# danihae/bio-image-unet

Measured on AMD Instinct MI355X. Metric: voxels/sec fwd+bwd, higher is better.
Workload: dtype bf16; 1 GPU; cfg4: UNet3D(in_channels=1, out_channels=1, n_filter=32) input (4, 1, 128, 128, 128) per GPU, train step = forward + reference loss + backward + Adam; parallelism=dp1

## Files before the change

bio_image_unet_amd/_lib.py:

```python
from __future__ import annotations

import ctypes as C
import os

import torch

_HERE = os.path.dirname(os.path.abspath(__file__))
LIB_PATH = os.environ.get("BIU_LIB_PATH") or os.path.join(_HERE, "libbiu_hip.so")

BIU_F32, BIU_BF16 = 0, 1
BN_MAX_PARTIALS = 1024


class BiuError(RuntimeError):
    pass


class biu_act(C.Structure):
    _fields_ = [("p", C.c_void_p), ("n", C.c_int32), ("d", C.c_int32), ("h", C.c_int32), ("w", C.c_int32),
                ("c", C.c_int32), ("pitch", C.c_int32)]


class biu_pack_job(C.Structure):
    _fields_ = [("w", C.c_void_p), ("packed", C.c_void_p), ("transposed", C.c_int32), ("kind", C.c_int32), ("cin", C.c_int32),
                ("cout", C.c_int32), ("kd", C.c_int32), ("kh", C.c_int32), ("kw", C.c_int32), ("reserved", C.c_int32)]


class biu_xform(C.Structure):
    _fields_ = [("scale", C.c_void_p), ("shift", C.c_void_p), ("slope", C.c_void_p)]


class biu_mo2d_term(C.Structure):
    _fields_ = [("kind", C.c_int32), ("nb", C.c_int32), ("partial_off", C.c_longlong), ("numel", C.c_longlong), ("pixels", C.c_longlong),
                ("p0", C.c_float), ("p1", C.c_float), ("p2", C.c_float), ("weight", C.c_float)]


class biu_aug_params(C.Structure):
    _fields_ = [("flags", C.c_uint32), ("rot_k", C.c_uint32), ("blur_k", C.c_uint32), ("index", C.c_uint32), ("m", C.c_double * 6),
                ("alpha", C.c_float), ("beta", C.c_float), ("noise_a", C.c_float), ("noise_b", C.c_float),
                ("angle", C.c_float), ("scale", C.c_float), ("dx", C.c_float), ("dy", C.c_float)]


class biu_augf_params(C.Structure):
    _fields_ = [("flags", C.c_uint32), ("rot_k", C.c_uint32), ("blur_k", C.c_uint32), ("index", C.c_uint32), ("m", C.c_double * 6),
                ("cos_t", C.c_float), ("sin_t", C.c_float), ("alpha", C.c_float), ("beta", C.c_float), ("shot_s", C.c_float),
                ("gauss_sigma", C.c_float), ("angle", C.c_float), ("scale", C.c_float), ("dx", C.c_float), ("dy", C.c_float)]


_P = C.c_void_p
_A = C.POINTER(biu_act)
_X = C.POINTER(biu_xform)
_I = C.c_int
_F = C.c_float
_D = C.c_double
_Z = C.c_size_t

SIGNATURES = {
    "biu_last_error": (C.c_char_p, []),
    "biu_version": (_I, []),
    "biu_set_fp32_products": (_I, [_I]),
    "biu_set_fp32_products_3d": (_I, [_I]),
    "biu_conv_packed_bytes": (_Z, [_I, _I, _I, _I, _I, _I, _I, _I]),
    "biu_conv_pack": (_I, [_I, _P, _I, _I, _I, _I, _I, _I, _P, _P]),
    "biu_pack_batch": (_I, [_P, _I, _I, _P]),
    "biu_conv_split_workspace": (_Z, [_I, _A, _A, _I, _I, _I, _I, _I]),
    "biu_conv_fwd": (_I, [_A, _X, _P, _P, _P, _I, _I, _I, _I, _A, _P, _Z, _I, _P]),
    "biu_conv_fwd_stats_floats": (_Z, [_A, _I]),
    "biu_conv_fwd_stats": (_I, [_A, _X, _P, _P, _P, _I, _I, _I, _I, _A, _P, _Z, C.POINTER(C.c_int), _P, _Z, _I, _P]),
    "biu_conv_bwd_data": (_I, [_A, _P, _P, _I, _I, _I, _I, _A, _I, _P, _Z, _I, _P]),
    "biu_bwd_data_bnred_floats": (_Z, [_A, _I, _I]),
    "biu_conv_bwd_data_bnred": (_I, [_A, _P, _P, _I, _I, _I, _I, _A, _A, _P, _P, _P, _P, _P, _P, _Z, C.POINTER(C.c_int), _P, _Z, _I, _P]),
    "biu_convt_bwd_data_bnred": (_I, [_A, _P, _P, _I, _A, _A, _P, _P, _P, _P, _P, _P, _Z, C.POINTER(C.c_int), _I, _P]),
    "biu_conv_bwd_weight_workspace": (_Z, [_I, _I, _I, _I, _I, _I]),
    "biu_conv_bwd_weight": (_I, [_A, _X, _A, _I, _I, _I, _I, _P, _P, _P, _Z, _I, _P]),
    "biu_conv_bwd_weight_bn": (_I, [_A, _X, _A, _A, _P, _P, _P, _P, _P, _P, _I, _I, _I, _I, _P, _P, _Z, _I, _P]),
    "biu_bn_stats": (_I, [_A, _P, C.POINTER(C.c_int), _I, _P]),
    "biu_bn_finalize": (_I, [_P, _I, _I, _D, _P, _P, _P, _P, _F, _F, _P, _P, _P, _P, _P]),
    "biu_bn_eval_affine": (_I, [_I, _P, _P, _P, _P, _F, _P, _P, _P]),
    "biu_xform_apply": (_I, [_A, _X, _A, _I, _P]),
    "biu_bn_bwd_reduce": (_I, [_A, _A, _P, _P, _P, _P, _P, _P, C.POINTER(C.c_int), _I, _P]),
    "biu_bn_bwd_finalize": (_I, [_P, _I, _I, _D, _P, _P, _P, _P, _P, _P, _P, _P, _P]),
    "biu_bn_bwd_finalize_eval": (_I, [_P, _I, _I, _P, _P, _P, _P, _P, _P, _P, _P]),
    "biu_bn_bwd_apply": (_I, [_A, _A, _P, _P, _P, _P, _P, _P, _A, _I, _P]),
    "biu_maxpool_fwd": (_I, [_A, _X, _A, _I, _P]),
    "biu_maxpool_bwd": (_I, [_A, _X, _A, _A, _I, _I, _P]),
    "biu_maxpool_bwd_bnred": (_I, [_A, _X, _A, _A, _I, _P, _P, _P, _Z, C.POINTER(C.c_int), _I, _P]),
    "biu_nearest_down_fwd": (_I, [_A, _X, _A, _I, _P]),
    "biu_nearest_down_bwd": (_I, [_A, _A, _I, _I, _P]),
    "biu_nearest_up_fwd": (_I, [_A, _X, _A, _I, _P]),
    "biu_upconv_ok": (_I, [_A, _A, _I]),
    "biu_upconv_packed_bytes": (_Z, [_I, _I, _I, _I]),
    "biu_upconv_pack": (_I, [_I, _P, _I, _I, _I, _P, _P]),
    "biu_upconv_bwd_data": (_I, [_A, _P, _A, _I, _I, _P]),
    "biu_upconv_bwd_weight_workspace": (_Z, [_I, _I, _I]),
    "biu_upconv_bwd_weight_bn": (_I, [_A, _X, _A, _A, _P, _P, _P, _P, _P, _P, _P, _P, _Z, _I, _P]),
    "biu_upconv_fwd_stats_floats": (_Z, [_A, _A]),
    "biu_upconv_fwd": (_I, [_A, _X, _P, _P, _A, _P, _Z, C.POINTER(C.c_int), _I, _P]),
    "biu_nearest_up_bwd": (_I, [_A, _A, _I, _I, _P]),
    "biu_bce_dice_blocks": (_I, [C.c_longlong]),
    "biu_bce_dice_fwd": (_I, [_P, _P, _I, C.c_longlong, _P, _P]),
    "biu_bce_dice_bwd": (_I, [_P, _P, _I, C.c_longlong, _P, _P, _I, _P]),
    "biu_pair_smooth_l1_blocks": (_I, [C.c_longlong]),
    "biu_pair_smooth_l1_fwd": (_I, [_P, _I, C.c_longlong, _P, _P]),
    "biu_pair_smooth_l1_bwd": (_I, [_P, _I, C.c_longlong, _P, _P, _I, _P]),
    "biu_seg_loss_finish": (_I, [_P, _I, _I, C.c_longlong, _P, _I, _F, _F, _F, _I, _F, _F, _F, _I, _F, _P, _P]),
    "biu_seg_loss_coef": (_I, [_P, _P, _I, C.c_longlong, _F, _F, _F, _I, _F, _F, _F, _I, _F, _P, _P, _P]),
    "biu_head_dlogits": (_I, [_P, _P, _P, _I, _I, _I, C.c_longlong, _P, _I, _I, _P]),
    "biu_mo2d_loss_blocks": (_I, [C.c_longlong]),
    "biu_mo2d_loss_fwd": (_I, [_I, _F, _F, _P, _I, _P, _I, _I, _I, _I, _P, _P]),
    "biu_mo2d_loss_finish": (_I, [_P, _I, _P, _P, _P]),
    "biu_mo2d_loss_coef": (_I, [_P, _I, _P, _P, _P, _P]),
    "biu_mo2d_loss_bwd": (_I, [_I, _F, _F, _P, _I, _P, _I, _I, _I, _I, _P, _P, _P]),
    "biu_trilinear_up_fwd": (_I, [_A, _X, _A, _I, _P]),
    "biu_trilinear_up_bwd": (_I, [_A, _A, _I, _I, _P]),
    "biu_bilinear_up_fwd": (_I, [_A, _X, _A, _I, _P]),
    "biu_bilinear_up_bwd": (_I, [_A, _A, _I, _I, _P]),
    "biu_xcorr_fwd": (_I, [_A, _X, _A, _X, _A, _I, _P]),
    "biu_xcorr_bwd": (_I, [_A, _X, _A, _X, _A, _A, _A, _I, _I, _P]),
    "biu_conv_cat_ok": (_I, [_A, _A, _A, _I, _I, _I, _I, _I]),
    "biu_conv_fwd_cat": (_I, [_A, _X, _A, _X, _P, _P, _P, _I, _I, _I, _I, _A, _P, _Z, C.POINTER(C.c_int), _P, _Z, _I, _P]),
    "biu_conv_bwd_data_cat": (_I, [_A, _P, _P, _I, _I, _I, _I, _A, _I, _A, _I, _P, _Z, _I, _P]),
    "biu_conv_bwd_weight_cat": (_I, [_A, _X, _A, _X, _A, _A, _P, _P, _P, _P, _P, _P, _I, _I, _I, _I, _P, _P, _Z, _I, _P]),
    "biu_convt_packed_bytes": (_Z, [_I, _I, _I, _I, _I]),
    "biu_convt_pack": (_I, [_I, _P, _I, _I, _I, _I, _P, _P]),
    "biu_foldt_ok": (_I, [_A, _A, _A, _I]),
    "biu_foldt_packed_bytes": (_Z, [_I, _I, _I, _I]),
    "biu_foldt_pack": (_I, [_P, _P, _P, _P, _I, _I, _I, _I, _I, _P, _P]),
    "biu_foldt_fwd_stats_floats": (_Z, [_A, _A]),
# ... 94 lines not shown
```

bio_image_unet_amd/csrc/biu_api.hip:

```cpp
#include "biu_common.h"
#include "biu_internal.h"

#include <stdlib.h>
#include <string.h>

static const char* const kOffTokens[] = {
    "conv_fwd", "conv_dgrad", "conv_wgrad", "convt_fwd", "convt_dgrad", "convt_wgrad", "convt_all", "c1", "c1_mfma", "cat",
    "fused_stats", "wgrad_bn", "dgrad_bnred", "pool_pair", "pool_pipe", "pool_bnred", "head_bnred", "ksplit", "m16", "m16x2", "rr16",
    "wroll", "wroll16", "wroll2d", "upconv", "foldt", "foldall", "foldck8", "foldgemm", "croll", "froll", "prepack", "wsplitbn",
    "capturefork", "sidechain",
};
constexpr int kNumOffTokens = sizeof(kOffTokens) / sizeof(kOffTokens[0]);
static_assert(kNumOffTokens <= 64, "BiuEnv::off holds one bit per token");

static int off_index(const char* tok, size_t n) {
    for (int i = 0; i < kNumOffTokens; ++i)
        if (strlen(kOffTokens[i]) == n && strncmp(kOffTokens[i], tok, n) == 0) return i;
    return -1;
}
static void env_unknown(const char* var, const char* val, int n) {
    fprintf(stderr, "[biu] %s: unknown %s '%.*s' ignored\n", var, strcmp(var, "BIU_DISABLE") == 0 ? "token" : "value", n, val);
}
static bool parse_int(const char* s, int* v) {
    char* end = nullptr;
    const long r = strtol(s, &end, 10);
    if (end == s || *end) return false;
    *v = (int)r;
    return true;
}

const BiuEnv& biu_env() {
    static const BiuEnv env = [] {
        BiuEnv v{0, false, false, 0, 2, 0, 128};
        if (const char* p = getenv("BIU_DISABLE")) {
            while (true) {
                const size_t n = strcspn(p, ",");
                const int i = off_index(p, n);
                if (i >= 0) v.off |= 1ull << i;
                else if (n > 0) env_unknown("BIU_DISABLE", p, (int)n);
                if (!p[n]) break;
                p += n + 1;
            }
        }
        if (const char* e = getenv("BIU_ROLL"); e && *e) {
            if (strcmp(e, "always") == 0) v.roll_always = true;
            else env_unknown("BIU_ROLL", e, (int)strlen(e));
        }
        if (const char* e = getenv("BIU_FOLDT"); e && *e) {
            int n = 0;
            if (strcmp(e, "always") == 0) v.foldt_always = true;
            else if (strncmp(e, "cmax:", 5) == 0 && parse_int(e + 5, &n) && n > 0) v.foldt_cmax = n;
            else if (strcmp(e, "size") != 0) env_unknown("BIU_FOLDT", e, (int)strlen(e));
        }
        if (const char* e = getenv("BIU_FP32_PRODUCTS"); e && *e) {
            if (strcmp(e, "exact") == 0) v.fp32_products = 0;
            else if (strcmp(e, "bf16x3") == 0) v.fp32_products = 1;
            else if (strcmp(e, "bf16x6") != 0) env_unknown("BIU_FP32_PRODUCTS", e, (int)strlen(e));
        }
        if (const char* e = getenv("BIU_FP32_PRODUCTS_3D"); e && *e) {
            if (strcmp(e, "bf16x3") == 0) v.fp32_products_3d = 1;
            else if (strcmp(e, "bf16x6") == 0) v.fp32_products_3d = 2;
            else if (strcmp(e, "exact") != 0) env_unknown("BIU_FP32_PRODUCTS_3D", e, (int)strlen(e));
        }
// ... 192 lines not shown
        return a > b ? a : b;
    }
    return biu_mfma_wgrad_workspace(cin, cout, kd, kh, kw, dtype);
}

extern "C" int biu_conv_bwd_weight(const biu_act* x, const biu_xform* xf, const biu_act* dy, int kd, int kh, int kw,
                                   int dilation, float* dw, float* dbias, void* ws, size_t ws_bytes, int dtype,
                                   biu_stream stream) {
    BIU_REQUIRE(conv_args_ok(x, dy, kd, kh, kw, dilation), BIU_ERR_SHAPE, "conv_bwd_weight: x/dy extents differ");
    BIU_REQUIRE(dw, BIU_ERR_SHAPE, "conv_bwd_weight: null dw");
    if (!biu_off("c1") && biu_c1m_ok(x, dy, kd, kh, kw, dilation, dtype) && ws && ws_bytes >= biu_c1m_wgrad_workspace(dy->c, kd)) {
        int rc = biu_c1m_wgrad(x, xf, dy, nullptr, kd, dw, ws, ws_bytes, (hipStream_t)stream);
        if (rc == BIU_OK && dbias) rc = biu_chan_sum(dy, dbias, dtype, (hipStream_t)stream);
        return rc;
    }
    if (!biu_off("c1") && biu_c1_conv_ok(x, dy, kd, kh, kw, dilation, dtype) && ws && ws_bytes >= biu_c1_wgrad_workspace(dy->c, kd)) {
        int rc = biu_c1_conv_wgrad(x, xf, dy, kd, dw, ws, ws_bytes, dtype, (hipStream_t)stream);
        if (rc == BIU_OK && dbias) rc = biu_chan_sum(dy, dbias, dtype, (hipStream_t)stream);
        return rc;
    }
    if (!biu_off("conv_wgrad") && biu_mfma_wgrad_ok(x, dy, kd, kh, kw, dilation, dtype)) {
        BIU_REQUIRE(ws && ws_bytes >= biu_mfma_wgrad_workspace(x->c, dy->c, kd, kh, kw, dtype), BIU_ERR_WORKSPACE,
                    "conv_bwd_weight: workspace too small");
        return biu_mfma_wgrad(x, xf, dy, kd, kh, kw, dw, dbias, ws, ws_bytes, dtype, (hipStream_t)stream);
    }
    warn_slow_path("conv_bwd_weight", x, dy, kd * kh * kw);
    return biu_conv_bwd_weight_direct(x, xf, dy, kd, kh, kw, dilation, dw, dbias, dtype, (hipStream_t)stream);
}

extern "C" int biu_conv_bwd_weight_bn(const biu_act* x, const biu_xform* xf, const biu_act* da, const biu_act* y,
                                      const float* scale, const float* shift, const float* slope, const float* coefA,
                                      const float* coefB, const float* coefC, int kd, int kh, int kw, int dilation,
                                      float* dw, void* ws, size_t ws_bytes, int dtype, biu_stream stream) {
    BIU_REQUIRE(conv_args_ok(x, da, kd, kh, kw, dilation) && valid_act(y) && same_space(y, da) && y->c == da->c, BIU_ERR_SHAPE,
                "conv_bwd_weight_bn: extents differ");
    BIU_REQUIRE(dw && scale && shift && coefA && coefB && coefC, BIU_ERR_SHAPE, "conv_bwd_weight_bn: null pointer");
    const size_t es = dsize(dtype);
    const bool yok = ((uintptr_t)y->p % 16) == 0 && ((size_t)y->pitch * es) % 16 == 0 &&
                     (i64)y->d * y->h * y->w * y->pitch * (i64)es < (1LL << 32) - 65536;
    if (!biu_off("c1") && !biu_off("wgrad_bn") && yok && biu_c1m_ok(x, da, kd, kh, kw, dilation, dtype) && ws &&
        ws_bytes >= biu_c1m_wgrad_workspace(da->c, kd)) {
        BnBwdFuse bn{y, scale, shift, slope, coefA, coefB, coefC};
        return biu_c1m_wgrad(x, xf, da, &bn, kd, dw, ws, ws_bytes, (hipStream_t)stream);
    }
    if (!biu_off("conv_wgrad") && !biu_off("wgrad_bn") && yok && biu_mfma_wgrad_ok(x, da, kd, kh, kw, dilation, dtype)) {
        BIU_REQUIRE(ws && ws_bytes >= biu_mfma_wgrad_workspace(x->c, da->c, kd, kh, kw, dtype), BIU_ERR_WORKSPACE,
                    "conv_bwd_weight_bn: workspace too small");
        BnBwdFuse bn{y, scale, shift, slope, coefA, coefB, coefC};
        return biu_mfma_wgrad(x, xf, da, kd, kh, kw, dw, nullptr, ws, ws_bytes, dtype, (hipStream_t)stream, &bn);
    }
    int rc = biu_bn_bwd_apply(da, y, scale, shift, slope, coefA, coefB, coefC, da, dtype, stream);
    if (rc != BIU_OK) return rc;
    return biu_conv_bwd_weight(x, xf, da, kd, kh, kw, dilation, dw, nullptr, ws, ws_bytes, dtype, stream);
}

extern "C" int biu_conv_cat_ok(const biu_act* x0, const biu_act* x1, const biu_act* y, int kd, int kh, int kw, int dilation, int dtype) {
    if (!x0 || !x1 || !y || !valid_act(x0) || !valid_act(x1) || !valid_act(y) || !same_space(x0, y) || !same_space(x1, y)) return 0;
    if (biu_off("conv_fwd") || biu_off("conv_dgrad") || biu_off("conv_wgrad") || biu_off("cat")) return 0;
    return biu_mfma_conv_cat_ok(x0, x1, y, kd, kh, kw, dilation, dtype) ? 1 : 0;
}
extern "C" int biu_conv_fwd_cat(const biu_act* x0, const biu_xform* xf0, const biu_act* x1, const biu_xform* xf1, const float* w,
                                const void* packed, const float* bias, int kd, int kh, int kw, int dilation, const biu_act* y,
                                float* bn_partial, size_t bn_partial_floats, int* bn_nblk, void* ws, size_t ws_bytes, int dtype,
                                biu_stream stream) {
    BIU_REQUIRE(biu_conv_cat_ok(x0, x1, y, kd, kh, kw, dilation, dtype) && w && packed, BIU_ERR_UNSUPPORTED,
                "conv_fwd_cat: shapes not served by the two-source kernels (ask biu_conv_cat_ok)");
    ConvCat cat{x1, xf1, nullptr, 0};
    if (bn_partial && will_split(x0->c + x1->c, y, nullptr, kd, dtype, ws, ws_bytes)) {
        BIU_REQUIRE(bn_nblk, BIU_ERR_SHAPE, "conv_fwd_cat: null bn_nblk");
        int rc = biu_mfma_conv(x0, xf0, packed, bias, kd, kh, kw, y, 0, nullptr, dtype, (hipStream_t)stream, nullptr, &cat, ws, ws_bytes);
        if (rc != BIU_OK) return rc;
        BIU_REQUIRE(bn_partial_floats >= (size_t)BIU_BN_MAX_PARTIALS * y->c * 2, BIU_ERR_WORKSPACE, "conv_fwd_cat: partial buffer too small");
        return biu_bn_stats(y, bn_partial, bn_nblk, dtype, stream);
    }
    if (bn_partial) {
        BIU_REQUIRE(bn_nblk, BIU_ERR_SHAPE, "conv_fwd_cat: null bn_nblk");
        const int nb = dtype == BIU_F32 ? biu_mfma_conv_stat_rows(y, kd, x0, dtype, false, x0->c + x1->c) : biu_mfma_conv_stat_rows(y, kd);
        BIU_REQUIRE((size_t)nb * y->c * 2 <= bn_partial_floats, BIU_ERR_WORKSPACE, "conv_fwd_cat: partial buffer too small");
        int rc = biu_mfma_conv(x0, xf0, packed, bias, kd, kh, kw, y, 0, bn_partial, dtype, (hipStream_t)stream, nullptr, &cat);
        if (rc == BIU_OK) *bn_nblk = nb;
        return rc;
    }
    return biu_mfma_conv(x0, xf0, packed, bias, kd, kh, kw, y, 0, nullptr, dtype, (hipStream_t)stream, nullptr, &cat, ws, ws_bytes);
}
extern "C" int biu_conv_bwd_data_cat(const biu_act* dy, const float* w, const void* packed, int kd, int kh, int kw, int dilation,
                                     const biu_act* dx0, int accumulate0, const biu_act* dx1, int accumulate1, void* ws, size_t ws_bytes,
                                     int dtype, biu_stream stream) {
    BIU_REQUIRE(biu_conv_cat_ok(dx0, dx1, dy, kd, kh, kw, dilation, dtype) && w && packed, BIU_ERR_UNSUPPORTED,
                "conv_bwd_data_cat: shapes not served by the two-source kernels (ask biu_conv_cat_ok)");
    ConvCat cat{nullptr, nullptr, dx1, accumulate1};
    return biu_mfma_conv(dy, nullptr, packed, nullptr, kd, kh, kw, dx0, accumulate0, nullptr, dtype, (hipStream_t)stream, nullptr, &cat, ws, ws_bytes);
}
extern "C" int biu_conv_bwd_weight_cat(const biu_act* x0, const biu_xform* xf0, const biu_act* x1, const biu_xform* xf1,
                                       const biu_act* da, const biu_act* y, const float* scale, const float* shift,
                                       const float* slope, const float* coefA, const float* coefB, const float* coefC, int kd,
                                       int kh, int kw, int dilation, float* dw, void* ws, size_t ws_bytes, int dtype,
                                       biu_stream stream) {
    BIU_REQUIRE(biu_conv_cat_ok(x0, x1, da, kd, kh, kw, dilation, dtype) && dw, BIU_ERR_UNSUPPORTED,
                "conv_bwd_weight_cat: shapes not served by the two-source kernels (ask biu_conv_cat_ok)");
    BIU_REQUIRE(ws && ws_bytes >= biu_mfma_wgrad_workspace(x0->c + x1->c, da->c, kd, kh, kw, dtype), BIU_ERR_WORKSPACE,
                "conv_bwd_weight_cat: workspace too small");
    if (y) {
        const size_t es = dsize(dtype);
        BIU_REQUIRE(valid_act(y) && same_space(y, da) && y->c == da->c && scale && shift && coefA && coefB && coefC, BIU_ERR_SHAPE,
                    "conv_bwd_weight_cat: BatchNorm operands missing");
        BIU_REQUIRE(((uintptr_t)y->p % 16) == 0 && ((size_t)y->pitch * es) % 16 == 0 && (i64)y->d * y->h * y->w * y->pitch * (i64)es < (1LL << 32) - 65536,
// ... 198 lines not shown
```

bio_image_unet_amd/csrc/biu_conv_mfma.hip:

```cpp
#include "biu_internal.h"
#include <type_traits>
#include <cstring>
#include <mutex>
#include <cstdlib>

typedef float floatx16 __attribute__((ext_vector_type(16)));
typedef float floatx4 __attribute__((ext_vector_type(4)));
typedef __bf16 bf16x8 __attribute__((ext_vector_type(8)));

template <typename T> struct Frag;
template <> struct Frag<bf16_t> {
    static constexpr int PE = 8;
    __device__ static __forceinline__ void mma(const uint4& a, const uint4& b, floatx16& c) {
        c = __builtin_amdgcn_mfma_f32_32x32x16_bf16(__builtin_bit_cast(bf16x8, a), __builtin_bit_cast(bf16x8, b), c, 0, 0, 0);
    }
    __device__ static __forceinline__ void unpack(const uint4& v, float* f) {
        const unsigned u[4] = {v.x, v.y, v.z, v.w};
#pragma unroll
        for (int i = 0; i < 4; ++i) {
            f[2 * i] = __uint_as_float(u[i] << 16);
            f[2 * i + 1] = __uint_as_float(u[i] & 0xffff0000u);
        }
    }
    __device__ static __forceinline__ uint4 pack(const float* f) {
// ... 2262 lines not shown
    if (rc == BIU_OK) rc = mfma_pack_strided(1, w_conv + (size_t)cup * 27, ccat, cskip, cout, 3, 3, 3, dtype, base + b.sdg, st);
    return rc;
}
static bool foldt_roll_ok(const biu_act* x_low, const biu_act* skip, const biu_act* y, int dtype) {
    return !biu_off("froll") && skip && biu_fold_roll_ok(x_low, y, dtype) && biu_conv_roll_ok(skip, y, dtype, false, 1, false);
}
int biu_mfma_foldt_form(const biu_act* x_low, const biu_act* skip, const biu_act* y, int dtype) { return foldt_roll_ok(x_low, skip, y, dtype) ? 1 : 0; }
int biu_mfma_foldt_stat_rows(const biu_act* x_low, const biu_act* y, const biu_act* skip, int dtype) {
    if (skip && foldt_roll_ok(x_low, skip, y, dtype)) return biu_conv_roll_rows(skip, y, dtype);
    return biu_mfma_upconv_stat_rows(x_low, y);
}
int biu_mfma_foldt_fwd(const biu_act* x_low, const biu_xform* xf_low, const biu_act* skip, const biu_xform* xf_skip, const void* packed, const biu_act* y,
                       float* bn_partial, int dtype, hipStream_t st) {
    const FoldtBlob b = foldt_blob(x_low->c, skip->c, y->c, dtype);
    const char* base = (const char*)packed;
    if (foldt_roll_ok(x_low, skip, y, dtype)) {
        int rc = biu_fold_roll(x_low, xf_low, base + b.fwd, (const float*)(base + b.bias), (const float*)(base + b.fix), y, st);
        if (rc != BIU_OK) return rc;
        return biu_mfma_conv(skip, xf_skip, base + b.sfwd, nullptr, 3, 3, 3, y, 1, bn_partial, dtype, st, nullptr, nullptr, nullptr, 0);
    }
    int rc = biu_mfma_conv(skip, xf_skip, base + b.sfwd, (const float*)(base + b.bias), 3, 3, 3, y, 0, nullptr, dtype, st, nullptr, nullptr, nullptr, 0);
    if (rc != BIU_OK) return rc;
    const ShellDims sh = shell_dims(y->n, y->d, y->h, y->w);
    BIU_DISPATCH_DTYPE(dtype, hipLaunchKernelGGL(k_foldt_border_fix<T>, dim3(2048), dim3(256), 0, st, (char*)y->p,
                                                 sh, y->c, y->pitch, (const float*)(base + b.fix)));
    BIU_CHECK_LAUNCH("foldt_border_fix");
    return biu_mfma_upconv_fwd(x_low, xf_low, base + b.fwd, nullptr, y, bn_partial, dtype, st, 1);
}

typedef __bf16 bf16x4 __attribute__((ext_vector_type(4)));

struct WgradArgs {
    const char* pa;
    const char* pb;
    float* ws;
    const float* as_; const float* ab_; const float* al_;
    const float* bs_; const float* bb_; const float* bl_;
    int apitch, bpitch;
    int N, CA, CB;
    int GD, GH, GW;
    int BD, BH, BW;
    int nbd, nbh, nbw, nbricks;
    int njt;
    int jt_begin, jt_count;
    int write_back;
    unsigned long long* diag;
    const char* pb1; int bpitch1; int bsplit;
    const float* bs1_; const float* bb1_; const float* bl1_;
    int bricks_per_block;
    const char* py;
    int ypitch;
    const float* bn_scale; const float* bn_shift; const float* bn_slope;
    const float* bn_cA; const float* bn_cB; const float* bn_cC;
    float* dbias_out;
    int fold_par;
    size_t fold_slice_f;
};

template <typename T, int PE>
__device__ __forceinline__ uint4 apply_xf16(uint4 v, const float* sc, const float* sh, const float* sl) {
    using F = Frag<T>;
    float f[PE];
    F::unpack(v, f);
    lrelu_affine<PE>(f, sc, sh, sl);
    return F::pack(f);
}


constexpr bool wgrad_tab_in_lds(size_t tile_bytes, int pieces) { return tile_bytes + (size_t)pieces * 512 * 4 <= 150 * 1024; }

template <typename T, int KD, int KHW, int S, int TD, int TH, int TW, int KSPLIT, int NI, bool RR16 = false, bool FALL = false>
__global__ __launch_bounds__(512, 2) void k_wgrad_pipe(WgradArgs a) {
    using F = Frag<T>;
    constexpr int NTHR = 512, NWAVE = 8;
    constexpr int PE = F::PE;
    constexpr int CT = 32;
    constexpr int PPV = CT / PE;
    constexpr int XP = SplitOf<T>::parts;
    constexpr bool X3 = XP > 0;
    constexpr bool BFM = sizeof(T) == 2 || X3;
    constexpr int LES = BFM ? 2 : 4;
    constexpr int NPL = X3 ? XP : 1;
    constexpr int CTA = CT * NI, PPVA = CTA / PE, RSA = CTA * LES;
    constexpr int PD = (KD == 3) ? 1 : 0;
    constexpr int PHW = (KHW == 3) ? 1 : 0;
    constexpr bool FOLD = (KD == 2 && KHW == 2 && S == 1);
    constexpr int SD = (KD == 1) ? 1 : S;
    static_assert(!FALL || (FOLD && KSPLIT == 8 && NI == 1 && sizeof(T) == 2), "the all-parity form: bf16 fold, one wave per parity class");
    constexpr int HD = (TD - 1) * SD + (FALL ? 3 : KD), HH = (TH - 1) * S + (FALL ? 3 : KHW), HW = (TW - 1) * S + (FALL ? 3 : KHW);
    constexpr int HV = HD * HH * HW;
    constexpr int BVR = TD * TH * TW;
    constexpr int BV = FALL ? 8 * BVR : BVR;
    constexpr int TAPS = KD * KHW * KHW;
    constexpr int WPQ = NWAVE / KSPLIT;
    constexpr int IPW = (TAPS + WPQ - 1) / WPQ;
    static_assert(NWAVE % KSPLIT == 0, "K split must divide the wave count");
    constexpr int RS = CT * LES;
    constexpr int NA = (BV * PPVA + NTHR - 1) / NTHR;
    constexpr int NB = (HV * PPV + NTHR - 1) / NTHR;
    constexpr int KUNIT = BFM ? 16 : 2;
    constexpr int NKG = BV / KUNIT;
    static_assert(TW % 16 == 0 && NKG % KSPLIT == 0, "brick / split mismatch");

    extern __shared__ __attribute__((aligned(16))) uint4 lds[];
    char* at = (char*)lds;
    char* bt = at + NPL * BV * RSA;
// ... 591 lines not shown
    float* wsp = a.ws + (FALL ? (size_t)wave * a.fold_slice_f : (size_t)0);
    if (jj < a.CB) {
#pragma unroll
        for (int t2 = 0; t2 < IPW; ++t2) {
            const int tap = tapid[t2];
            if (tap < TAPS) {
#pragma unroll
                for (int ni = 0; ni < NI; ++ni)
#pragma unroll
                    for (int e = 0; e < 16; ++e) {
                        const int ii = it * CTA + ni * CT + (e & 3) + 8 * (e >> 2) + 4 * hf;
                        if (ii < a.CA) atomicAdd(wsp + ((size_t)tap * a.CA + ii) * a.CB + jj, acc[t2][ni][e]);
                    }
            }
        }
    }
}

typedef unsigned v4u_t __attribute__((ext_vector_type(4)));
__device__ __forceinline__ void bload_lds16(unsigned voff, v4u_t rsrc, unsigned lds_base_uniform) {
    unsigned keep;
    asm volatile("s_mov_b32 %0, m0\n\ts_mov_b32 m0, %3\n\ts_nop 0\n\tbuffer_load_dwordx4 %1, %2, 0 offen lds\n\ts_mov_b32 m0, %0"
                 : "=&s"(keep)
                 : "v"(voff), "s"(rsrc), "s"(lds_base_uniform)
                 : "memory");
}
__device__ __forceinline__ v4u_t raw_rsrc(const void* base, unsigned bytes) {
    const unsigned long long pa = (unsigned long long)base;
    v4u_t r;
    r[0] = __builtin_amdgcn_readfirstlane((unsigned)pa);
    r[1] = __builtin_amdgcn_readfirstlane((unsigned)(pa >> 32) & 0xffffu);
    r[2] = __builtin_amdgcn_readfirstlane(bytes);
    r[3] = 0x00020000u;
    return r;
}

#ifndef BIU_WROLL_ABL
#define BIU_WROLL_ABL 0
#endif
#ifndef BIU_DIAG_WAVE
#define BIU_DIAG_WAVE 0
#endif
constexpr int WR_TD = 2, WR_TH = 8, WR_TW = 16;
constexpr int WR_HH = WR_TH + 2, WR_HW = WR_TW + 2, WR_PL = WR_HH * WR_HW;
constexpr int WR_RS = 64;
constexpr int WR_PLB = WR_PL * WR_RS;
constexpr int WR_NBI = 24;
constexpr int WR_PAIRB = WR_NBI * 1024;
constexpr int WR_NPAIR = 4;
constexpr int WR_BV = WR_TD * WR_TH * WR_TW;
constexpr int WR_AB = WR_BV * WR_RS;
constexpr int WR_NAI = WR_AB / 1024;
constexpr int WR_NABUF = 3;
constexpr size_t WR_LDS = (size_t)WR_NPAIR * WR_PAIRB + WR_NABUF * WR_AB + 9 * 32 * sizeof(float);

__device__ __forceinline__ unsigned opaque_s(unsigned x) { asm volatile("" : "+s"(x)); return x; }
template <int N> __device__ __forceinline__ void wait_vmcnt() { asm volatile("s_waitcnt vmcnt(%0)" ::"n"(N) : "memory"); }

template <bool BNF, bool K2D, bool A16 = false>
__global__ __launch_bounds__(512, 2) void k_wgrad_roll(WgradArgs a) {
    static_assert(!(K2D && A16), "the 16-channel plain operand form exists for volumes only");
    using T = bf16_t;
    using F = Frag<T>;
    constexpr int TD = WR_TD, TH = WR_TH, TW = WR_TW, HW = WR_HW, PL = WR_PL, RS = WR_RS, PLB = WR_PLB, PAIRB = WR_PAIRB;
    constexpr int CT = 32, PE = 8, TAPS = K2D ? 9 : 27, IPW = K2D ? 3 : 4, NROW = TD * TH;
    constexpr int NBK = WR_NBI / 8, NAK = A16 ? 1 : WR_NAI / 8;
    constexpr int NACC = A16 ? 6 : IPW;

    extern __shared__ __attribute__((aligned(16))) uint4 lds[];
    char* bring = (char*)lds;
    char* abuf = bring + WR_NPAIR * PAIRB;
    float* lxf = (float*)(abuf + WR_NABUF * WR_AB);
    constexpr int LB = 0, LBN = 3 * CT;

    const int tid = threadIdx.x, lane = tid & 63;
    const int wave = __builtin_amdgcn_readfirstlane(tid >> 6);
    const int it = blockIdx.y / a.jt_count, jt = a.jt_begin + blockIdx.y % a.jt_count;
    const int piece = lane & 3;
    const int apc = A16 ? (piece & 1) : piece;
    const int ac0 = it * CT + apc * PE, bc0 = jt * CT + piece * PE;
    const bool apiece_ok = ac0 < a.CA, bpiece_ok = bc0 < a.CB;
    const bool b_src1 = a.pb1 && jt * CT >= a.bsplit;
    const char* pb_ = b_src1 ? a.pb1 : a.pb;
    const int bpitch_ = b_src1 ? a.bpitch1 : a.bpitch;
    const int bc_local = bc0 - (b_src1 ? a.bsplit : 0);
    const float* bs_ = b_src1 ? a.bs1_ : a.bs_;
    const float* bb_ = b_src1 ? a.bb1_ : a.bb_;
    const float* bl_ = b_src1 ? a.bl1_ : a.bl_;
    const bool b_xf = bs_ != nullptr;
    constexpr bool bn_fused = BNF;
    const bool wb = bn_fused && a.write_back;
    if (tid < CT && bn_fused) {
        const int ca = it * CT + tid;
        const bool ok = ca < a.CA;
        lxf[LBN + 0 * CT + tid] = ok ? a.bn_scale[ca] : 1.f;
        lxf[LBN + 1 * CT + tid] = ok ? a.bn_shift[ca] : 0.f;
        lxf[LBN + 2 * CT + tid] = (ok && a.bn_slope) ? a.bn_slope[ca] : 1.f;
        lxf[LBN + 3 * CT + tid] = ok ? a.bn_cA[ca] : 0.f;
        lxf[LBN + 4 * CT + tid] = ok ? a.bn_cB[ca] : 0.f;
        lxf[LBN + 5 * CT + tid] = ok ? a.bn_cC[ca] : 0.f;
    }
    if (tid < CT) {
        const int cb = jt * CT + tid;
        const int cbl = cb - (b_src1 ? a.bsplit : 0);
        lxf[LB + 0 * CT + tid] = (b_xf && cb < a.CB) ? bs_[cbl] : 1.f;
        lxf[LB + 1 * CT + tid] = (b_xf && cb < a.CB) ? bb_[cbl] : 0.f;
        lxf[LB + 2 * CT + tid] = (b_xf && cb < a.CB) ? bl_[cbl] : 1.f;
    }

    floatx16 acc[NACC];
#pragma unroll
    for (int t = 0; t < NACC; ++t)
#pragma unroll
        for (int e = 0; e < 16; ++e) acc[t][e] = 0.f;
    const int wkd = wave / 3, wkw = wave % 3;
    const bool has_x = A16 ? (wave < 4) : (!K2D && wave < 3);
    int tapid[IPW];
#pragma unroll
    for (int t = 0; t < IPW; ++t) {
        if constexpr (K2D) tapid[t] = (wave < 6) ? t * 3 + wkw : TAPS;
        else tapid[t] = (t < 3) ? (wkd * 3 + t) * 3 + wkw : (has_x ? (2 * 3 + wave) * 3 + 2 : TAPS);
    }
    int ab_lane;
    {
        const int g = lane >> 4, li = lane & 15, qrow = li >> 2, p = li & 3, cg = g & 1, h = g >> 1;
        ab_lane = (8 * h + qrow) * RS + (16 * cg + 4 * p) * 2;
    }

    unsigned bco[NBK], aco[NAK];
#pragma unroll
    for (int k = 0; k < NBK; ++k) {
        const int v = ((wave + 8 * k) * 64 + lane) >> 2;
        const int pl = v / PL, r = v % PL;
        bco[k] = (v < 2 * PL && bpiece_ok) ? (unsigned)(pl | ((r / HW) << 10) | ((r % HW) << 20)) : 0xffffffffu;
    }
#pragma unroll
    for (int k = 0; k < NAK; ++k) {
        const int v = ((wave + 8 * k) * 64 + lane) >> 2;
        if constexpr (A16) aco[k] = apiece_ok ? (unsigned)((piece >> 1) | ((v >> 4) << 10) | ((v & 15) << 20)) : 0xffffffffu;
        else aco[k] = apiece_ok ? (unsigned)((v >> 7) | (((v >> 4) & 7) << 10) | ((v & 15) << 20)) : 0xffffffffu;
    }
    const unsigned rowA = (unsigned)a.apitch * 2u, rowY = (unsigned)a.ypitch * 2u, rowB = (unsigned)bpitch_ * 2u;
    const size_t sampA = (size_t)a.GD * a.GH * a.GW * rowA, sampY = (size_t)a.GD * a.GH * a.GW * rowY, sampB = (size_t)a.BD * a.BH * a.BW * rowB;
    const unsigned lds0 = (unsigned)(uintptr_t)((__attribute__((address_space(3))) void*)bring);

    int cn = 0, ch0 = 0, cw0 = 0;
    v4u_t rsB, rsA;
    __amdgpu_buffer_rsrc_t rsAr, rsYr;
    struct Slot { unsigned bmask, amask; uint4 pa[BNF ? NAK : 1], pyv[BNF ? NAK : 1]; };
    Slot sl0, sl1;
    sl0.bmask = sl0.amask = sl1.bmask = sl1.amask = 0;
    unsigned bbase[NBK], abase_[NAK], ybase_[BNF ? NAK : 1];
    unsigned planeB = 0, planeA = 0, planeY = 0;
    auto set_column = [&](int col) __attribute__((always_inline)) {
        int c = col;
        const int wb_ = c % a.nbw; c /= a.nbw;
        const int hb = c % a.nbh;
        cn = c / a.nbh;
        ch0 = hb * TH; cw0 = wb_ * TW;
        rsB = raw_rsrc(pb_ + (size_t)cn * sampB, (unsigned)sampB);
        rsA = raw_rsrc(a.pa + (size_t)cn * sampA, (unsigned)sampA);
        rsAr = __builtin_amdgcn_make_buffer_rsrc((void*)(a.pa + (size_t)cn * sampA), 0, (int)(unsigned)sampA, 0x00020000);
        rsYr = __builtin_amdgcn_make_buffer_rsrc((void*)(a.py + (size_t)cn * sampY), 0, bn_fused ? (int)(unsigned)sampY : 0, 0x00020000);
        planeB = (unsigned)(a.BH * a.BW) * rowB; planeA = (unsigned)(a.GH * a.GW) * rowA; planeY = (unsigned)(a.GH * a.GW) * rowY;
#pragma unroll
        for (int k = 0; k < NBK; ++k) {
            const unsigned x = bco[k];
            const int gh = ch0 - 1 + (int)((x >> 10) & 1023u), gw = cw0 - 1 + (int)(x >> 20);
            const bool ok = x != 0xffffffffu && (unsigned)gh < (unsigned)a.BH && (unsigned)gw < (unsigned)a.BW;
            bbase[k] = ok ? (unsigned)(gh * a.BW + gw) * rowB + (unsigned)bc_local * 2u + (x & 1023u) * planeB : 0xffffffffu;
        }
#pragma unroll
        for (int k = 0; k < NAK; ++k) {
            const unsigned x = aco[k];
            const int gh = ch0 + (int)((x >> 10) & 1023u), gw = cw0 + (int)(x >> 20);
            const bool ok = x != 0xffffffffu && gh < a.GH && gw < a.GW;
            const unsigned vox = (unsigned)(gh * a.GW + gw);
            abase_[k] = ok ? vox * rowA + (unsigned)ac0 * 2u + (x & 1023u) * planeA : 0xffffffffu;
            if constexpr (BNF) ybase_[k] = ok ? vox * rowY + (unsigned)ac0 * 2u + (x & 1023u) * planeY : 0xffffffffu;
        }
    };
    struct FetchCtx { int pair, buf; bool bd0, bd1, ad0, ad1; unsigned dofB, dofA, dofY; };
    auto fetch_ctx = [&](int pair, int gp0, int buf, int d0) __attribute__((always_inline)) -> FetchCtx {
        FetchCtx f;
        f.pair = pair; f.buf = buf;
        f.bd0 = (unsigned)gp0 < (unsigned)a.BD; f.bd1 = (unsigned)(gp0 + 1) < (unsigned)a.BD;
        f.ad0 = d0 < a.GD; f.ad1 = d0 + 1 < a.GD;
        f.dofB = opaque_s((unsigned)gp0 * planeB);
        f.dofA = opaque_s((unsigned)d0 * planeA); f.dofY = opaque_s((unsigned)d0 * planeY);
        f.pair = (int)opaque_s((unsigned)pair); f.buf = (int)opaque_s((unsigned)buf);
        return f;
    };
    auto fetch_piece = [&](Slot& sl, const FetchCtx& f, int i) __attribute__((always_inline)) {
        if (i < NBK) {
            const int k = i;
            const bool ok = bbase[k] != 0xffffffffu && ((bco[k] & 1u) ? f.bd1 : f.bd0);
            bload_lds16(ok ? bbase[k] + f.dofB : 0xffffffffu, rsB, lds0 + (unsigned)(f.pair * PAIRB + (wave + 8 * k) * 1024));
            sl.bmask = (k == 0 ? 0u : sl.bmask) | (ok ? (1u << k) : 0u);
        } else {
            const int k = i - NBK;
            const bool ok = abase_[k] != 0xffffffffu && ((aco[k] & 1u) ? f.ad1 : f.ad0);
            if constexpr (BNF) {
                const auto v0 = __builtin_amdgcn_raw_buffer_load_b128(rsAr, ok ? (int)(abase_[k] + f.dofA) : -1, 0, 0);
                const auto v1 = __builtin_amdgcn_raw_buffer_load_b128(rsYr, ok ? (int)(ybase_[k] + f.dofY) : -1, 0, 0);
                sl.pa[k] = make_uint4(v0[0], v0[1], v0[2], v0[3]);
                sl.pyv[k] = make_uint4(v1[0], v1[1], v1[2], v1[3]);
            } else {
                bload_lds16(ok ? abase_[k] + f.dofA : 0xffffffffu, rsA, lds0 + (unsigned)(WR_NPAIR * PAIRB + f.buf * WR_AB + (wave + 8 * k) * 1024));
            }
            sl.amask = (k == 0 ? 0u : sl.amask) | (ok ? (1u << k) : 0u);
        }
    };
    auto fetch_all = [&](Slot& sl, const FetchCtx& f, bool with_a) __attribute__((always_inline)) {
#pragma unroll
        for (int i = 0; i < NBK + NAK; ++i)
            if (i < NBK || with_a) fetch_piece(sl, f, i);
    };
    auto finish = [&](Slot& sl, int pair_, int buf_, int d0, bool with_a) __attribute__((always_inline)) {
        const int pair = (int)opaque_s((unsigned)pair_), buf = (int)opaque_s((unsigned)buf_);
        const unsigned dofA = opaque_s((unsigned)d0 * planeA);
        if (b_xf) {
            float sc[PE], sh[PE], sl_[PE];
#pragma unroll
            for (int e = 0; e < PE; ++e) { sc[e] = lxf[LB + piece * PE + e]; sh[e] = lxf[LB + CT + piece * PE + e]; sl_[e] = lxf[LB + 2 * CT + piece * PE + e]; }
#pragma unroll
            for (int k = 0; k < NBK; ++k) {
                if ((sl.bmask >> k) & 1u) {
                    uint4* p_ = (uint4*)(bring + pair * PAIRB + (wave + 8 * k) * 1024 + lane * 16);
                    *p_ = apply_xf16<T, PE>(*p_, sc, sh, sl_);
                }
            }
        }
        __builtin_amdgcn_sched_barrier(0);
        if constexpr (BNF) if (with_a) {
            {
                float ks[PE], kh[PE], kl[PE];
#pragma unroll
                for (int e = 0; e < PE; ++e) { ks[e] = lxf[LBN + apc * PE + e]; kh[e] = lxf[LBN + CT + apc * PE + e]; kl[e] = lxf[LBN + 2 * CT + apc * PE + e]; }
#pragma unroll
                for (int k = 0; k < NAK; ++k) {
                    if ((sl.amask >> k) & 1u) {
                        float g[PE], yy[PE];
                        F::unpack(sl.pa[k], g);
                        F::unpack(sl.pyv[k], yy);
#pragma unroll
                        for (int e = 0; e < PE; ++e) g[e] *= (fmaf(ks[e], yy[e], kh[e]) > 0.f ? 1.f : kl[e]);
                        sl.pa[k] = F::pack(g);
                    }
                }
            }
            __builtin_amdgcn_sched_barrier(0);
            {
                float ka[PE], kb[PE], kc[PE];
#pragma unroll
                for (int e = 0; e < PE; ++e) { ka[e] = lxf[LBN + 3 * CT + apc * PE + e]; kb[e] = lxf[LBN + 4 * CT + apc * PE + e]; kc[e] = lxf[LBN + 5 * CT + apc * PE + e]; }
#pragma unroll
                for (int k = 0; k < NAK; ++k) {
                    uint4 v = make_uint4(0, 0, 0, 0);
                    const bool ok = (sl.amask >> k) & 1u;
                    if (ok) {
                        float g[PE], yy[PE];
                        F::unpack(sl.pa[k], g);
                        F::unpack(sl.pyv[k], yy);
#pragma unroll
                        for (int e = 0; e < PE; ++e) g[e] = fmaf(ka[e], g[e], fmaf(kb[e], yy[e], kc[e]));
                        v = F::pack(g);
                    }
                    if (wb) __builtin_amdgcn_raw_buffer_store_b128(v4u_t{v.x, v.y, v.z, v.w}, rsAr, ok ? (int)(abase_[k] + dofA) : -1, 0, 0);
                    *(uint4*)(abuf + buf * WR_AB + (wave + 8 * k) * 1024 + lane * 16) = v;
                }
            }
        }
    };
    auto wait_older = [&](bool younger_in_flight) __attribute__((always_inline)) {
        if (!younger_in_flight) { wait_vmcnt<0>(); return; }
        if (wb) wait_vmcnt<NAK + NBK + 2 * NAK>();
        else if (bn_fused) wait_vmcnt<NBK + 2 * NAK>();
        else wait_vmcnt<NBK + NAK>();
    };

    typedef bf16x4 __attribute__((address_space(3))) * lp;
    auto rd = [&](const char* p_) -> bf16x8 {
        const bf16x4 v0 = __builtin_amdgcn_ds_read_tr16_b64_v4bf16((lp)(p_));
        const bf16x4 v1 = __builtin_amdgcn_ds_read_tr16_b64_v4bf16((lp)(p_ + 4 * RS));
        return __builtin_shufflevector(v0, v1, 0, 1, 2, 3, 4, 5, 6, 7);
    };
    auto mfma_step = [&](auto has_x_c, int s4, int buf, auto&& issue) __attribute__((always_inline)) {
        constexpr bool HAS_X = decltype(has_x_c)::value;
        auto pj = [&](int j) -> const char* { return bring + opaque_s((unsigned)(((s4 + (j >> 1)) & 3) * PAIRB + (j & 1) * PLB)); };
        if constexpr (A16) {
            const int uj = wave & 3, ukw = wave >> 2;
            const char* b0 = pj(uj) + ukw * RS + ab_lane;
            const char* c0 = pj(uj) + 2 * RS + ab_lane;
            const char* ab = abuf + opaque_s((unsigned)(buf * WR_AB)) + ab_lane;
            bf16x8 ring[4], ring2[HAS_X ? 4 : 1], faa[2];
            faa[0] = rd(ab);
// ... 141 lines not shown
    if (wdiag && (tid & 63) == 0 && (tid >> 6) == (BIU_DIAG_WAVE)) {
        for (int q_ = 0; q_ < 8; ++q_) atomicAdd(wdiag + q_, dsum_[q_]);
        atomicAdd(wdiag + 8, __builtin_readcyclecounter() - t0c_);
        atomicAdd(wdiag + 9, __builtin_amdgcn_s_memrealtime() - t0r_);
    }
#endif
    const int hf = lane >> 5;
    const int jj = jt * CT + (lane & 31);
    if constexpr (A16) {
        const int uj = wave & 3;
        if (jj < a.CB) {
#pragma unroll
            for (int u = 0; u < 2; ++u) {
                if (u == 1 && !has_x) break;
                const int kw = u ? 2 : (wave >> 2);
#pragma unroll
                for (int tb = 0; tb < 3; ++tb)
#pragma unroll
                    for (int e = 0; e < 16; ++e) {
                        const int kd = uj - (e >> 3), ii = (e & 3) + 8 * ((e >> 2) & 1) + 4 * hf;
                        if (kd >= 0 && kd <= 2 && ii < a.CA) atomicAdd(a.ws + ((size_t)((kd * 3 + tb) * 3 + kw) * a.CA + ii) * a.CB + jj, acc[u * 3 + tb][e]);
                    }
            }
        }
        return;
    }
    if (jj < a.CB) {
#pragma unroll
        for (int t2 = 0; t2 < IPW; ++t2) {
            const int tap = tapid[t2];
            if (tap < TAPS) {
#pragma unroll
                for (int e = 0; e < 16; ++e) {
                    const int ii = it * CT + (e & 3) + 8 * (e >> 2) + 4 * hf;
                    if (ii < a.CA) atomicAdd(a.ws + ((size_t)tap * a.CA + ii) * a.CB + jj, acc[t2][e]);
                }
            }
        }
    }
}

static bool wroll_fits(const WgradArgs& a) {
    const int ncols = a.N * ((a.GH + WR_TH - 1) / WR_TH) * ((a.GW + WR_TW - 1) / WR_TW);
    return a.GD >= 8 && ncols >= 8;
}
static bool wroll2d_fits(const WgradArgs& a, i64 bytesA, i64 bytesB, i64 bytesY) {
    const int ncols = ((a.GH + WR_TH - 1) / WR_TH) * ((a.GW + WR_TW - 1) / WR_TW);
    return a.N >= 8 && ncols >= 8 && a.CA * a.CB > 1024 && bytesA < BIU_MAX_SAMPLE_BYTES && bytesB < BIU_MAX_SAMPLE_BYTES && bytesY < BIU_MAX_SAMPLE_BYTES;
}

static int launch_wgrad_roll(WgradArgs a, hipStream_t st, bool k2d = false) {
    if (k2d) { a.GD = a.BD = a.N; a.N = 1; }
    const bool a16 = !k2d && a.CA == 16 && !biu_off("wroll16");
    a.nbd = 1;
    a.nbh = (a.GH + WR_TH - 1) / WR_TH;
    a.nbw = (a.GW + WR_TW - 1) / WR_TW;
    const int ncols = a.N * a.nbh * a.nbw;
    a.nbricks = ncols;
    const int nit = (a.CA + 31) / 32;
    a.njt = (a.CB + 31) / 32;
    a.bricks_per_block = 0;
#ifdef BIU_DIAG
    a.diag = biu_diag_buffer;
#else
    a.diag = nullptr;
#endif
    static bool attr_set = false;
    if (!attr_set) {
        if (hipFuncSetAttribute((const void*)k_wgrad_roll<false, false>, hipFuncAttributeMaxDynamicSharedMemorySize, (int)WR_LDS) != hipSuccess ||
            hipFuncSetAttribute((const void*)k_wgrad_roll<true, false>, hipFuncAttributeMaxDynamicSharedMemorySize, (int)WR_LDS) != hipSuccess ||
            hipFuncSetAttribute((const void*)k_wgrad_roll<false, true>, hipFuncAttributeMaxDynamicSharedMemorySize, (int)WR_LDS) != hipSuccess ||
            hipFuncSetAttribute((const void*)k_wgrad_roll<true, true>, hipFuncAttributeMaxDynamicSharedMemorySize, (int)WR_LDS) != hipSuccess ||
            hipFuncSetAttribute((const void*)k_wgrad_roll<false, false, true>, hipFuncAttributeMaxDynamicSharedMemorySize, (int)WR_LDS) != hipSuccess ||
            hipFuncSetAttribute((const void*)k_wgrad_roll<true, false, true>, hipFuncAttributeMaxDynamicSharedMemorySize, (int)WR_LDS) != hipSuccess)
            return biu_fail(BIU_ERR_LAUNCH, "wgrad_roll: cannot reserve %zu bytes of LDS", WR_LDS);
        attr_set = true;
    }
    auto launch = [&](int jt_begin, int jt_count, int write_back, bool with_bn) {
        WgradArgs b = a;
        if (!with_bn) b.py = nullptr;
        b.jt_begin = jt_begin; b.jt_count = jt_count; b.write_back = write_back;
        const int pairs = nit * jt_count;
        int g = num_cus() / pairs;
        if (g >= 16) g = grid_per_column(num_cus(), pairs);
        if (g < 1) g = 1;
        if (g > ncols) g = ncols;
        if (k2d) {
            if (with_bn) hipLaunchKernelGGL((k_wgrad_roll<true, true>), dim3(g, pairs), dim3(512), WR_LDS, st, b);
            else hipLaunchKernelGGL((k_wgrad_roll<false, true>), dim3(g, pairs), dim3(512), WR_LDS, st, b);
        } else if (a16) {
            if (with_bn) hipLaunchKernelGGL((k_wgrad_roll<true, false, true>), dim3(g, pairs), dim3(512), WR_LDS, st, b);
            else hipLaunchKernelGGL((k_wgrad_roll<false, false, true>), dim3(g, pairs), dim3(512), WR_LDS, st, b);
        } else {
            if (with_bn) hipLaunchKernelGGL((k_wgrad_roll<true, false>), dim3(g, pairs), dim3(512), WR_LDS, st, b);
            else hipLaunchKernelGGL((k_wgrad_roll<false, false>), dim3(g, pairs), dim3(512), WR_LDS, st, b);
        }
    };
    if (a.py && a.njt > 1) {
        launch(0, 1, 1, true);
        BIU_CHECK_LAUNCH("wgrad_roll");
        launch(1, a.njt - 1, 0, false);
    } else {
        launch(0, a.njt, a.py ? 1 : 0, a.py != nullptr);
    }
    BIU_CHECK_LAUNCH("wgrad_roll");
    return BIU_OK;
}

__global__ void k_wgrad_finalize(const float* __restrict__ ws, int rows, int cols, int taps, float* __restrict__ dw, int ld_cols = 0, int c_off = 0) {
    const size_t total = (size_t)rows * cols * taps;
    for (size_t i = (size_t)blockIdx.x * blockDim.x + threadIdx.x; i < total; i += (size_t)gridDim.x * blockDim.x) {
        const int tap = (int)(i % taps);
        const size_t r = i / taps;
        const int c = (int)(r % cols);
        const int rr = (int)(r / cols);
        const size_t o = ld_cols > 0 ? ((size_t)rr * ld_cols + c_off + c) * taps + tap : i;
        dw[o] = ws[((size_t)tap * rows + rr) * cols + c];
    }
}

__global__ void k_zero_f32(float* __restrict__ p, size_t n, float* __restrict__ q, int nq) {
    for (size_t i = (size_t)blockIdx.x * blockDim.x + threadIdx.x; i < n; i += (size_t)gridDim.x * blockDim.x) p[i] = 0.f;
    if (q && blockIdx.x == 0)
        for (int i = threadIdx.x; i < nq; i += blockDim.x) q[i] = 0.f;
}
static int zero_ws(void* ws, size_t bytes, float* extra, int nextra, hipStream_t st) {
    const size_t n = bytes / sizeof(float);
    hipLaunchKernelGGL(k_zero_f32, dim3(grid_for((i64)n, 256, 1024)), dim3(256), 0, st, (float*)ws, n, extra, nextra);
    if (hipGetLastError() != hipSuccess) return biu_fail(BIU_ERR_LAUNCH, "wgrad: zero-fill launch failed");
    return BIU_OK;
}

static bool wgrad_chan_ok(int cin, int cout) { return cin >= 16 && cin % 8 == 0 && cout >= 16 && cout % 8 == 0; }

static size_t wgrad_acc_bytes(int cin, int cout, int taps) { return (((size_t)cin * cout * taps * sizeof(float)) + 255) & ~(size_t)255; }

size_t biu_mfma_wgrad_workspace(int cin, int cout, int kd, int kh, int kw, int dtype) {
    if (!wgrad_chan_ok(cin, cout)) return 0;
    const size_t red = biu_chan_sum_workspace(cout);
    if (kh == 3 && kw == 3 && (kd == 1 || kd == 3)) return wgrad_acc_bytes(cin, cout, kd * 9) + red;
    if (kh == 2 && kw == 2 && (kd == 1 || kd == 2)) return wgrad_acc_bytes(cin, cout, kd * 4) + red;
    return 0;
}

// ... 25 lines not shown
    constexpr int NA_ = (BV * PPV_ * NI + 511) / 512, NB_ = (HV * PPV_ + 511) / 512;
    const size_t tile_bytes = (size_t)(HV + BV * NI) * 32 * (SplitOf<T>::parts ? 2 * SplitOf<T>::parts : sizeof(T));
    const size_t lds_bytes = tile_bytes + (3 + 9 * NI) * 32 * sizeof(float) + (wgrad_tab_in_lds(tile_bytes, NA_ + NB_) ? (size_t)(NA_ + NB_) * 512 * sizeof(unsigned) : 0);
    a.nbd = (a.GD + TD - 1) / TD;
    a.nbh = (a.GH + TH - 1) / TH;
    a.nbw = (a.GW + TW - 1) / TW;
    a.nbricks = a.N * a.nbd * a.nbh * a.nbw;
    const int nit = (a.CA + 32 * NI - 1) / (32 * NI);
    a.njt = (a.CB + 31) / 32;
    a.bricks_per_block = 0;
    auto kern = k_wgrad_pipe<T, KD, KHW, S, TD, TH, TW, KSPLIT, NI, RR16, FALL>;
    static bool attr_set = false;
    if (!attr_set) {
        if (hipFuncSetAttribute((const void*)kern, hipFuncAttributeMaxDynamicSharedMemorySize, (int)lds_bytes) != hipSuccess)
            return biu_fail(BIU_ERR_LAUNCH, "wgrad_pipe: cannot reserve %zu bytes of LDS", lds_bytes);
        attr_set = true;
    }
    auto launch = [&](int jt_begin, int jt_count, int write_back, bool with_bn) {
        WgradArgs b = a;
#ifdef BIU_DIAG
        b.diag = biu_diag_buffer;
#else
        b.diag = nullptr;
#endif
        if (!with_bn) b.py = nullptr;
        b.jt_begin = jt_begin; b.jt_count = jt_count; b.write_back = write_back;
        const int pairs = nit * jt_count;
        int g = num_cus() / pairs;
        if (g >= 16) g = grid_per_column(num_cus(), pairs);
        if (g < 1) g = 1;
        if (g > b.nbricks) g = b.nbricks;
        hipLaunchKernelGGL(kern, dim3(g, pairs), dim3(512), lds_bytes, st, b);
    };
    if (a.py && a.njt > 1) {
        launch(0, 1, 1, true);
        BIU_CHECK_LAUNCH("wgrad_pipe");
        launch(1, a.njt - 1, 0, false);
    } else {
        launch(0, a.njt, a.py ? 1 : 0, a.py != nullptr);
    }
    BIU_CHECK_LAUNCH("wgrad_pipe");
    return BIU_OK;
}

static int wgrad_xf(const biu_xform* xf, const float** s, const float** b, const float** l) {
    const bool has = xf && (xf->scale || xf->shift || xf->slope);
    if (has) BIU_REQUIRE(xf->scale && xf->shift && xf->slope, BIU_ERR_UNSUPPORTED, "wgrad_mfma: partial biu_xform");
    *s = has ? xf->scale : nullptr;
    *b = has ? xf->shift : nullptr;
    *l = has ? xf->slope : nullptr;
    return BIU_OK;
}

int biu_mfma_wgrad(const biu_act* x, const biu_xform* xf, const biu_act* dy, int kd, int kh, int kw, float* dw, float* dbias,
                   void* ws, size_t ws_bytes, int dtype, hipStream_t st, const BnBwdFuse* bn, const biu_act* x1, const biu_xform* xf1,
                   int dw_ld_cols, int dw_c_off) {
    WgradArgs a;
    int rc_ = BIU_OK;
    if (bn && !biu_off("wsplitbn") && dtype == BIU_BF16 && kd == 3 && x->c + (x1 ? x1->c : 0) > 32 && nvox(dy) <= 4 * 32 * 32 * 32) {
        rc_ = biu_bn_bwd_apply(dy, bn->y, bn->scale, bn->shift, bn->slope, bn->cA, bn->cB, bn->cC, dy, dtype, (biu_stream)st);
        if (rc_ != BIU_OK) return rc_;
        bn = nullptr;
    }
    if (bn) {
        a.py = (const char*)bn->y->p; a.ypitch = bn->y->pitch;
        a.bn_scale = bn->scale; a.bn_shift = bn->shift; a.bn_slope = bn->slope;
        a.bn_cA = bn->cA; a.bn_cB = bn->cB; a.bn_cC = bn->cC;
    } else {
        a.py = nullptr; a.ypitch = 0;
        a.bn_scale = a.bn_shift = a.bn_slope = a.bn_cA = a.bn_cB = a.bn_cC = nullptr;
    }
    a.pa = (const char*)dy->p;  a.apitch = dy->pitch;  a.CA = dy->c;
    a.pb = (const char*)x->p;   a.bpitch = x->pitch;   a.CB = x->c;
    a.dbias_out = nullptr;
    a.fold_par = -1;
    a.pb1 = nullptr; a.bpitch1 = 0; a.bsplit = 0; a.bs1_ = a.bb1_ = a.bl1_ = nullptr;
    if (x1) {
        a.pb1 = (const char*)x1->p; a.bpitch1 = x1->pitch; a.bsplit = x->c; a.CB = x->c + x1->c;
        rc_ = wgrad_xf(xf1, &a.bs1_, &a.bb1_, &a.bl1_);
        if (rc_) return rc_;
    }
    a.ws = (float*)ws;
    a.as_ = a.ab_ = a.al_ = nullptr;
    int rc = wgrad_xf(xf, &a.bs_, &a.bb_, &a.bl_);
    if (rc) return rc;
    a.N = x->n;
    a.GD = a.BD = x->d; a.GH = a.BH = x->h; a.GW = a.BW = x->w;
    const int taps = kd * 9;
    const size_t need = wgrad_acc_bytes(a.CA, a.CB, taps);
    BIU_REQUIRE(ws_bytes >= need + (dbias ? biu_chan_sum_workspace(dy->c) : 0), BIU_ERR_WORKSPACE, "wgrad_mfma: workspace %zu too small", ws_bytes);
    if (int zr = zero_ws(ws, need, nullptr, 0, st)) return zr;
    if (dtype == BIU_BF16 && kd == 3 && a.CB == 16 && !x1 && !biu_off("rr16")) rc = launch_wgrad<bf16_t, 3, 3, 1, 4, 8, 16, 1, 1, true>(a, st);
    else if (dtype == BIU_BF16 && kd == 3 && !biu_off("wroll") && wroll_fits(a)) rc = launch_wgrad_roll(a, st);
    else if (dtype == BIU_BF16 && kd == 1 && !biu_off("wroll") && !biu_off("wroll2d") &&
             wroll2d_fits(a, (i64)nvox(dy) * dy->pitch * 2, (i64)nvox(x) * x->pitch * 2 > (x1 ? (i64)nvox(x1) * x1->pitch * 2 : 0) ? (i64)nvox(x) * x->pitch * 2 : (i64)nvox(x1) * x1->pitch * 2,
                          bn ? (i64)nvox(bn->y) * bn->y->pitch * 2 : 0))
        rc = launch_wgrad_roll(a, st, true);
    else if (dtype == BIU_BF16) rc = (kd == 3) ? launch_wgrad<bf16_t, 3, 3, 1, 4, 8, 16, 1>(a, st) : launch_wgrad<bf16_t, 1, 3, 1, 1, 16, 32, 4>(a, st);
    else if (kd == 1 && x3_mode_of(kd, dtype) == 2) rc = launch_wgrad<f32x6_t, 1, 3, 1, 1, 16, 16, 4>(a, st);
    else if (kd == 1 && x3_mode_of(kd, dtype) == 1) rc = launch_wgrad<f32x3_t, 1, 3, 1, 1, 16, 16, 4>(a, st);
    else if (kd == 3 && x3_mode_of(kd, dtype) == 2) rc = launch_wgrad<f32x6_t, 3, 3, 1, 2, 4, 16, 1>(a, st);
    else if (kd == 3 && x3_mode_of(kd, dtype) == 1) rc = launch_wgrad<f32x3_t, 3, 3, 1, 2, 4, 16, 1>(a, st);
    else rc = (kd == 3) ? launch_wgrad<float, 3, 3, 1, 4, 4, 16, 1>(a, st) : launch_wgrad<float, 1, 3, 1, 1, 16, 16, 4>(a, st);
    if (rc != BIU_OK) return rc;
    hipLaunchKernelGGL(k_wgrad_finalize, dim3(grid_for((i64)a.CA * a.CB * taps, 256, 2048)), dim3(256), 0, st, (const float*)ws,
                       a.CA, a.CB, taps, dw, dw_ld_cols, dw_c_off);
    BIU_CHECK_LAUNCH("wgrad_finalize");
    if (dbias) return biu_chan_sum_vec(dy, dbias, (char*)ws + need, dtype, st);
    return BIU_OK;
}

__global__ void k_upconv_wgrad_unfold(const float* __restrict__ ws, size_t slice_f, int cout, int cin, float* __restrict__ dw) {
    const size_t total = (size_t)cout * cin * 27;
    for (size_t idx = (size_t)blockIdx.x * blockDim.x + threadIdx.x; idx < total; idx += (size_t)gridDim.x * blockDim.x) {
        const int k = (int)(idx % 27);
        const size_t r = idx / 27;
        const int ci = (int)(r % cin), co = (int)(r / cin);
        const int kk[3] = {k / 9, (k / 3) % 3, k % 3};
        float sum = 0.f;
        for (int p = 0; p < 8; ++p) {
            int t = 0;
#pragma unroll
            for (int ax = 0; ax < 3; ++ax) {
                const int pa = (p >> (2 - ax)) & 1;
                const int ta = pa == 0 ? (kk[ax] >= 1 ? 1 : 0) : (kk[ax] == 2 ? 1 : 0);
                t |= ta << (2 - ax);
            }
            sum += ws[(size_t)p * slice_f + ((size_t)t * cout + co) * cin + ci];
        }
        dw[idx] = sum;
    }
}
size_t biu_mfma_upconv_wgrad_workspace(int cin, int cout, int dtype) {
    if ((dtype != BIU_BF16 && dtype != BIU_F32) || !wgrad_chan_ok(cin, cout)) return 0;
    return 8 * wgrad_acc_bytes(cout, cin, 8);
}
int biu_mfma_upconv_wgrad(const biu_act* x, const biu_xform* xf, const biu_act* dy, float* dw, void* ws, size_t ws_bytes, int dtype,
                          hipStream_t st, const BnBwdFuse* bn) {
    WgradArgs a;
    if (bn) {
        a.py = (const char*)bn->y->p; a.ypitch = bn->y->pitch;
        a.bn_scale = bn->scale; a.bn_shift = bn->shift; a.bn_slope = bn->slope;
        a.bn_cA = bn->cA; a.bn_cB = bn->cB; a.bn_cC = bn->cC;
    } else {
        a.py = nullptr; a.ypitch = 0;
// ... 294 lines not shown
```

bio_image_unet_amd/csrc/biu_direct.hip:

```cpp
#include "biu_common.h"
#include "biu_internal.h"

thread_local char biu_errbuf[512] = {0};

int biu_fail(int code, const char* fmt, ...) {
    va_list ap;
    va_start(ap, fmt);
    vsnprintf(biu_errbuf, sizeof(biu_errbuf), fmt, ap);
    va_end(ap);
    return code;
}

extern "C" const char* biu_last_error(void) { return biu_errbuf; }
extern "C" int biu_version(void) { return 100; }
extern "C" int biu_set_fp32_products(int mode) { return biu_mfma_set_fp32_products(mode); }
extern "C" int biu_set_fp32_products_3d(int mode) { return biu_mfma_set_fp32_products_3d(mode); }

#define TPB 256

struct Vox {
    int n, d, h, w;
};
__device__ __forceinline__ Vox unvox(i64 v, int D, int H, int W) {
    Vox r;
// ... 1104 lines not shown
        }
    }
    BIU_DISPATCH_DTYPE(dtype, hipLaunchKernelGGL(k_head_fwd<T>, dim3(grid_for(nvox(x), TPB, 8192)), dim3(TPB), 0, st,
                                                 dact(x), dxf(xf), w, bias, cout, act, logits, activated));
    BIU_CHECK_LAUNCH("head_fwd");
    return BIU_OK;
}
extern "C" size_t biu_head_bwd_workspace(int cin) {
    size_t a = (size_t)BIU_BN_MAX_PARTIALS * cin * 2 * sizeof(float), b = biu_head_bwd_fused_workspace(cin);
    return a > b ? a : b;
}
extern "C" int biu_head_bwd(const biu_act* x, const biu_xform* xf, const float* w, int cout, const float* dlogits,
                            const biu_act* dx, float* dw, float* dbias, void* ws, size_t ws_bytes, int dtype,
                            biu_stream stream) {
    BIU_REQUIRE(valid_act(x) && w && dlogits && cout > 0 && cout <= HEAD_MAX_COUT, BIU_ERR_UNSUPPORTED, "head_bwd: bad arguments");
    hipStream_t st = (hipStream_t)stream;
    if (dx) BIU_REQUIRE(valid_act(dx) && same_space(x, dx) && dx->c == x->c, BIU_ERR_SHAPE, "head_bwd: dx shape mismatch");
    if (biu_head_bwd_fused_ok(x, dx, cout, dtype) && ws && ws_bytes >= biu_head_bwd_fused_workspace(x->c))
        return biu_head_bwd_fused(x, xf, w, cout, dlogits, dx, dw, dbias, ws, ws_bytes, dtype, st);
    if (dx) {
        i64 total = nvox(dx) * dx->c;
        BIU_DISPATCH_DTYPE(dtype, hipLaunchKernelGGL(k_head_bwd_data<T>, dim3(grid_for(total, TPB, 16384)), dim3(TPB), 0,
                                                     st, x->c, w, cout, dlogits, dact(dx)));
        BIU_CHECK_LAUNCH("head_bwd_data");
    }
    if (dw) {
        BIU_REQUIRE(ws && ws_bytes >= biu_head_bwd_workspace(x->c), BIU_ERR_WORKSPACE, "head_bwd: workspace too small");
        ReducePlan p = plan_reduce(nvox(x), x->c, BIU_BN_MAX_PARTIALS);
        i64 S = (i64)x->d * x->h * x->w;
        for (int o0 = 0; o0 < cout; o0 += 2) {
            BIU_DISPATCH_DTYPE(dtype, {
                HeadWgradF<T> f{dact(x), dxf(xf), dlogits, cout, o0, S};
                hipLaunchKernelGGL(k_chan_reduce2<HeadWgradF<T>>, dim3(p.nblk), dim3(TPB), 0, st, f, nvox(x), x->c, p.cw,
                                   p.vpb, (float*)ws);
            });
            BIU_CHECK_LAUNCH("head_wgrad");
            hipLaunchKernelGGL(k_partial_sum, dim3(x->c), dim3(TPB), 0, st, (const float*)ws, p.nblk, x->c,
                               dw + (i64)o0 * x->c, (o0 + 1 < cout) ? dw + (i64)(o0 + 1) * x->c : (float*)nullptr);
            BIU_CHECK_LAUNCH("partial_sum");
        }
    }
    if (dbias) {
        i64 S = (i64)x->d * x->h * x->w;
        hipLaunchKernelGGL(k_head_dbias, dim3(cout), dim3(TPB), 0, st, dlogits, x->n, cout, S, dbias);
        BIU_CHECK_LAUNCH("head_dbias");
    }
    return BIU_OK;
}

extern "C" int biu_head_bwd_bnred(const biu_act* x, const biu_xform* xf, const float* w, int cout, const float* dlogits,
                                  const biu_act* dx, float* dw, float* dbias, void* ws, size_t ws_bytes, const float* mean,
                                  const float* invstd, float* partial, size_t partial_floats, int* nblk, int dtype,
                                  biu_stream stream) {
    BIU_REQUIRE(valid_act(x) && w && dlogits && dx && valid_act(dx) && same_space(x, dx) && dx->c == x->c && cout > 0 &&
                    cout <= HEAD_MAX_COUT, BIU_ERR_SHAPE, "head_bwd_bnred: bad arguments");
    BIU_REQUIRE(xf && xf->scale && xf->shift && mean && invstd && partial && nblk, BIU_ERR_SHAPE, "head_bwd_bnred: null vector");
    BIU_REQUIRE(partial_floats >= (size_t)BIU_BN_MAX_PARTIALS * x->c * 2, BIU_ERR_WORKSPACE, "head_bwd_bnred: partial buffer too small");
    if (!biu_off("head_bnred") && biu_head_bwd_bnred_ok(x, dx, cout, dtype) && ws && ws_bytes >= biu_head_bwd_fused_workspace(x->c))
        return biu_head_bwd_bnred_fused(x, xf, w, cout, dlogits, dx, dw, dbias, ws, mean, invstd, partial, nblk, dtype, (hipStream_t)stream);
    int rc = biu_head_bwd(x, xf, w, cout, dlogits, dx, dw, dbias, ws, ws_bytes, dtype, stream);
    if (rc != BIU_OK) return rc;
    return biu_bn_bwd_reduce(dx, x, xf->scale, xf->shift, xf->slope, mean, invstd, partial, nblk, dtype, stream);
}

extern "C" int biu_max_join_fwd(const biu_act* a, const biu_xform* xa, const biu_act* b, const biu_xform* xb,
                                const biu_act* out, int dtype, biu_stream stream) {
    BIU_REQUIRE(valid_act(a) && valid_act(b) && valid_act(out) && same_space(a, b) && same_space(a, out) &&
                    a->c == b->c && a->c == out->c, BIU_ERR_SHAPE, "max_join_fwd: shape mismatch");
    hipStream_t st = (hipStream_t)stream;
    const int g = 16 / (int)dsize(dtype);
    bool ok = vec_ok(a, g, dtype) && vec_ok(b, g, dtype) && vec_ok(out, g, dtype);
    EW_LAUNCH(k_max_join_fwd, nvox(a) * a->c, ok, dact(a), dxf(xa), dact(b), dxf(xb), dact(out));
    BIU_CHECK_LAUNCH("max_join_fwd");
    return BIU_OK;
}
extern "C" int biu_max_join_bwd(const biu_act* a, const biu_xform* xa, const biu_act* b, const biu_xform* xb,
                                const biu_act* dout, const biu_act* da, const biu_act* db, int accumulate, int dtype,
                                biu_stream stream) {
    BIU_REQUIRE(valid_act(a) && valid_act(b) && valid_act(dout) && valid_act(da) && valid_act(db) && same_space(a, b) &&
                    same_space(a, dout) && same_space(a, da) && same_space(a, db) && a->c == b->c && a->c == dout->c &&
                    a->c == da->c && a->c == db->c, BIU_ERR_SHAPE, "max_join_bwd: shape mismatch");
    hipStream_t st = (hipStream_t)stream;
    const int g = 16 / (int)dsize(dtype);
    bool ok = vec_ok(a, g, dtype) && vec_ok(b, g, dtype) && vec_ok(dout, g, dtype) && vec_ok(da, g, dtype) && vec_ok(db, g, dtype);
    EW_LAUNCH(k_max_join_bwd, nvox(a) * a->c, ok, dact(a), dxf(xa), dact(b), dxf(xb), dact(dout), dact(da), dact(db), accumulate);
    BIU_CHECK_LAUNCH("max_join_bwd");
    return BIU_OK;
}
extern "C" int biu_act_add(const biu_act* src, const biu_act* dst, int accumulate, int dtype, biu_stream stream) {
    BIU_REQUIRE(valid_act(src) && valid_act(dst) && same_space(src, dst) && src->c == dst->c, BIU_ERR_SHAPE,
                "act_add: shape mismatch");
    hipStream_t st = (hipStream_t)stream;
    const int g = 16 / (int)dsize(dtype);
    bool ok = vec_ok(src, g, dtype) && vec_ok(dst, g, dtype);
    EW_LAUNCH(k_act_add, nvox(src) * src->c, ok, dact(src), dact(dst), accumulate);
    BIU_CHECK_LAUNCH("act_add");
    return BIU_OK;
}
extern "C" int biu_from_nchw(const float* src, const biu_act* dst, int dtype, biu_stream stream) {
    BIU_REQUIRE(src && valid_act(dst), BIU_ERR_SHAPE, "from_nchw: bad arguments");
    hipStream_t st = (hipStream_t)stream;
    i64 total = nvox(dst) * dst->c;
    BIU_DISPATCH_DTYPE(dtype, hipLaunchKernelGGL(k_from_nchw<T>, dim3(grid_for(total, TPB, 16384)), dim3(TPB), 0, st, src, dact(dst)));
    BIU_CHECK_LAUNCH("from_nchw");
    return BIU_OK;
}
extern "C" int biu_to_nchw(const biu_act* src, const biu_xform* xf, float* dst, int dtype, biu_stream stream) {
    BIU_REQUIRE(dst && valid_act(src), BIU_ERR_SHAPE, "to_nchw: bad arguments");
    hipStream_t st = (hipStream_t)stream;
    i64 total = nvox(src) * src->c;
    BIU_DISPATCH_DTYPE(dtype, hipLaunchKernelGGL(k_to_nchw<T>, dim3(grid_for(total, TPB, 16384)), dim3(TPB), 0, st, dact(src), dxf(xf), dst));
    BIU_CHECK_LAUNCH("to_nchw");
// ... 106 lines not shown
```

bio_image_unet_amd/csrc/biu_internal.h:

```cpp
#pragma once
#include "biu_common.h"

struct BiuEnv {
    unsigned long long off;
    bool roll_always;
    bool foldt_always;
    int foldt_cmax;
    int fp32_products;
    int fp32_products_3d;
    int fall_maxca;
};
const BiuEnv& biu_env();
bool biu_off(const char* token);

#define BIU_HIDDEN __attribute__((visibility("hidden")))
extern "C" BIU_HIDDEN int biu_conv_fwd_direct(const biu_act* x, const biu_xform* xf, const float* w, const float* bias, int kd,
                                   int kh, int kw, int dil, const biu_act* y, int dtype, hipStream_t st);
extern "C" BIU_HIDDEN int biu_conv_bwd_data_direct(const biu_act* dy, const float* w, int kd, int kh, int kw, int dil,
                                        const biu_act* dx, int accumulate, int dtype, hipStream_t st);
extern "C" BIU_HIDDEN int biu_conv_bwd_weight_direct(const biu_act* x, const biu_xform* xf, const biu_act* dy, int kd, int kh,
                                          int kw, int dil, float* dw, float* dbias, int dtype, hipStream_t st);
extern "C" BIU_HIDDEN int biu_convt_fwd_direct(const biu_act* x, const biu_xform* xf, const float* w, const float* bias, int kd,
                                    const biu_act* y, int dtype, hipStream_t st);
extern "C" BIU_HIDDEN int biu_convt_bwd_data_direct(const biu_act* dy, const float* w, int kd, const biu_act* dx, int accumulate,
                                         int dtype, hipStream_t st);
extern "C" BIU_HIDDEN int biu_convt_bwd_weight_direct(const biu_act* x, const biu_xform* xf, const biu_act* dy, int kd, float* dw,
                                           float* dbias, int dtype, hipStream_t st);
int biu_chan_sum(const biu_act* a, float* out, int dtype, hipStream_t st);
bool biu_convt_shapes_ok(const biu_act* lo, const biu_act* hi, int kd);

size_t biu_mfma_packed_bytes(int kind, int cin, int cout, int kd, int kh, int kw, int dilation, int dtype);
int biu_mfma_pack(int kind, const float* w, int cin, int cout, int kd, int kh, int kw, int dtype, void* packed,
                  hipStream_t st);
bool biu_mfma_conv_ok(const biu_act* x, const biu_act* y, int kd, int kh, int kw, int dilation, int dtype);
struct BnRedFuse {
    const biu_act* y;
    const float *scale, *shift, *slope, *mean, *invstd;
};
bool biu_mfma_conv_cat_ok(const biu_act* x0, const biu_act* x1, const biu_act* y, int kd, int kh, int kw, int dilation, int dtype);
struct ConvCat {
    const biu_act* x1; const biu_xform* xf1;
    const biu_act* y1; int accumulate1;
};
int biu_mfma_conv(const biu_act* x, const biu_xform* xf, const void* packed, const float* bias, int kd, int kh, int kw,
                  const biu_act* y, int accumulate, float* bn_partial, int dtype, hipStream_t st, const BnRedFuse* red = nullptr,
                  const ConvCat* cat = nullptr, void* split_ws = nullptr, size_t split_ws_bytes = 0);
bool biu_conv_roll_ok(const biu_act* x, const biu_act* y, int dtype, bool has_cat, int accumulate, bool red);
int biu_conv_roll_mshape(const biu_act* x, const biu_act* y, int dtype);
int biu_conv_roll_rows(const biu_act* x, const biu_act* y, int dtype);
int biu_conv_roll(const biu_act* x, const biu_xform* xf, const void* packed, const float* bias, const biu_act* y, float* bn_partial, const BnRedFuse* red,
                  hipStream_t st, int accumulate = 0);
bool biu_fold_roll_ok(const biu_act* x_low, const biu_act* y, int dtype);
int biu_fold_roll(const biu_act* x_low, const biu_xform* xf, const void* packed_fwd, const float* bias_sum, const float* fix, const biu_act* y, hipStream_t st);
size_t biu_fold_gemm_layout_floats(int cin_low, int cup, int cout);
bool biu_fold_gemm_ok(int cin_low, int cup, int cout);
int biu_fold_gemm_layouts(const float* w_conv, int ccat, int cup, int cout, const float* w_t, int cin_low, float* layouts, hipStream_t st);
int biu_fold_gemm_compose(const float* layouts, int cin_low, int cup, int cout, const float* b_t, float* wfold, float* wb, hipStream_t st);
int biu_fold_gemm_chain(const float* G, size_t slice_f, const float* layouts, int cin_low, int cup, int cout, int ccat, float* dw_conv, float* dw_t,
                        const float* b_t, const float* Sk, hipStream_t st);
size_t biu_mfma_conv_split_bytes(int cin, const biu_act* y, const biu_act* y1, int kd, int dtype);
int biu_mfma_convt_dgrad_bricks(const biu_act* dx, int kd);
int biu_mfma_convt_dgrad_rows(const biu_act* dx, int kd, int cdy, int dtype);
int biu_mfma_pack_batch(const biu_pack_job* jobs_device, int n, int dtype, hipStream_t st);
int biu_mfma_set_fp32_products(int mode);
int biu_mfma_set_fp32_products_3d(int mode);
int biu_mfma_conv_ksplit(int cin, const biu_act* y, int kd, int dtype);
int biu_mfma_conv_stat_rows(const biu_act* y, int kd, const biu_act* x = nullptr, int dtype = -1, bool red = false, int cin = -1);
int biu_mfma_conv_bricks(const biu_act* y, int kd, const biu_act* x = nullptr, int dtype = -1, int cin = -1);
size_t biu_mfma_wgrad_workspace(int cin, int cout, int kd, int kh, int kw, int dtype);
bool biu_mfma_wgrad_ok(const biu_act* x, const biu_act* dy, int kd, int kh, int kw, int dilation, int dtype);
struct BnBwdFuse {
    const biu_act* y;
    const float *scale, *shift, *slope, *cA, *cB, *cC;
};
int biu_mfma_wgrad(const biu_act* x, const biu_xform* xf, const biu_act* dy, int kd, int kh, int kw, float* dw,
                   float* dbias, void* ws, size_t ws_bytes, int dtype, hipStream_t st, const BnBwdFuse* bn = nullptr,
                   const biu_act* x1 = nullptr, const biu_xform* xf1 = nullptr, int dw_ld_cols = 0, int dw_c_off = 0);

size_t biu_mfma_convt_packed_bytes(int kind, int cin, int cout, int kd, int dtype);
int biu_mfma_convt_pack(int kind, const float* w, int cin, int cout, int kd, int dtype, void* packed, hipStream_t st);
bool biu_mfma_upconv_ok(const biu_act* x, const biu_act* y, int dtype);
size_t biu_mfma_upconv_packed_bytes(int kind, int cin, int cout, int dtype);
int biu_mfma_upconv_pack(int kind, const float* w, int cin, int cout, int dtype, void* packed, hipStream_t st, const float* wf = nullptr);
int biu_mfma_upconv_dgrad_rows(const biu_act* dx);
int biu_mfma_upconv_dgrad(const biu_act* dy, const void* packed, const biu_act* dx, int accumulate, int dtype, hipStream_t st, float* bn_partial = nullptr,
                          const BnRedFuse* red = nullptr);
struct BnBwdFuse;
size_t biu_mfma_upconv_wgrad_workspace(int cin, int cout, int dtype);
int biu_mfma_upconv_wgrad(const biu_act* x, const biu_xform* xf, const biu_act* dy, float* dw, void* ws, size_t ws_bytes, int dtype,
                          hipStream_t st, const BnBwdFuse* bn);
int biu_mfma_upconv_stat_rows(const biu_act* x, const biu_act* y);
int biu_mfma_upconv_fwd(const biu_act* x, const biu_xform* xf, const void* packed, const float* bias, const biu_act* y, float* bn_partial,
                        int dtype, hipStream_t st, int accumulate = 0);
bool biu_mfma_foldt_ok(const biu_act* x_low, const biu_act* skip, const biu_act* y, int dtype);
bool biu_mfma_foldt_worth(const biu_act* x_low, const biu_act* y);
size_t biu_mfma_foldt_packed_bytes(int cin_low, int cskip, int cout, int dtype);
int biu_mfma_foldt_pack(const float* w_conv, const float* b_conv, const float* w_t, const float* b_t, int cin_low, int cup, int cskip, int cout, int dtype,
                        void* packed, hipStream_t st);
int biu_mfma_foldt_stat_rows(const biu_act* x_low, const biu_act* y, const biu_act* skip = nullptr, int dtype = -1);
int biu_mfma_foldt_form(const biu_act* x_low, const biu_act* skip, const biu_act* y, int dtype);
int biu_mfma_foldt_fwd(const biu_act* x_low, const biu_xform* xf_low, const biu_act* skip, const biu_xform* xf_skip, const void* packed, const biu_act* y,
                       float* bn_partial, int dtype, hipStream_t st);
int biu_mfma_foldt_dgrad(const biu_act* dy, const void* packed, const biu_act* dx_low, int acc_low, const biu_act* dskip, int acc_skip, int dtype,
                         hipStream_t st, float* bn_partial_low, const BnRedFuse* red_low, void* ws, size_t ws_bytes);
size_t biu_mfma_foldt_wgrad_workspace(int cin_low, int cskip, int cout, int dtype);
int biu_mfma_foldt_wgrad(const biu_act* x_low, const biu_xform* xf_low, const biu_act* skip, const biu_xform* xf_skip, const biu_act* da, const BnBwdFuse* bn,
                         const float* dy_sum, const float* w_conv, const float* w_t, const float* b_t, int cup, float* dw_conv, float* dw_t, float* db_t, void* ws, size_t ws_bytes,
                         int dtype, hipStream_t st, int phases = 7);
bool biu_mfma_convt_ok(int kind, const biu_act* lo, const biu_act* hi, int kd, int dtype);
int biu_mfma_convt_fwd(const biu_act* x, const biu_xform* xf, const void* packed, const float* bias, int kd, const biu_act* y,
                       int dtype, hipStream_t st);
int biu_mfma_convt_dgrad(const biu_act* dy, const void* packed, int kd, const biu_act* dx, int accumulate, int dtype, hipStream_t st,
                         float* bn_partial = nullptr, const BnRedFuse* red = nullptr);
bool biu_mfma_convt_wgrad_ok(const biu_act* x, const biu_act* dy, int kd, int dtype);
int biu_mfma_convt_wgrad(const biu_act* x, const biu_xform* xf, const biu_act* dy, int kd, float* dw, float* dbias, void* ws,
                         size_t ws_bytes, int dtype, hipStream_t st);

bool biu_c1_conv_ok(const biu_act* x, const biu_act* y, int kd, int kh, int kw, int dil, int dtype);
int biu_c1_conv_fwd(const biu_act* x, const biu_xform* xf, const float* w, const float* bias, int kd, const biu_act* y, int dtype, hipStream_t st);
size_t biu_c1_wgrad_workspace(int cout, int kd);
int biu_c1_conv_wgrad(const biu_act* x, const biu_xform* xf, const biu_act* dy, int kd, float* dw, void* ws, size_t ws_bytes, int dtype, hipStream_t st);
bool biu_vec_reduce_ok(const biu_act* a, int dtype);
int biu_bn_stats_vec(const biu_act* y, float* partial, int* nblk_out, int dtype, hipStream_t st);
int biu_bn_bwd_reduce_vec(const biu_act* da, const biu_act* y, const float* scale, const float* shift, const float* slope,
                          const float* mean, const float* invstd, float* partial, int* nblk_out, int dtype, hipStream_t st);
size_t biu_chan_sum_workspace(int c);
int biu_chan_sum_vec(const biu_act* a, float* out, void* ws, int dtype, hipStream_t st);
// ... 32 lines not shown
```

bio_image_unet_amd/csrc/biu_special.hip:

```cpp
#include "biu_internal.h"
#include <cstring>
#include <cstdlib>
#include <stdlib.h>

#define TPB 256

struct Vox4 { int n, d, h, w; };
__device__ __forceinline__ Vox4 unvox4(i64 v, int D, int H, int W) {
    Vox4 r;
    if ((unsigned long long)v < (1ull << 32)) {
        unsigned u = (unsigned)v;
        r.w = (int)(u % (unsigned)W); u /= (unsigned)W;
        r.h = (int)(u % (unsigned)H); u /= (unsigned)H;
        r.d = (int)(u % (unsigned)D); u /= (unsigned)D;
        r.n = (int)u;
        return r;
    }
    r.w = (int)(v % W); v /= W;
    r.h = (int)(v % H); v /= H;
    r.d = (int)(v % D); v /= D;
    r.n = (int)v;
    return r;
}

// ... 429 lines not shown
int biu_bn_stats_vec(const biu_act* y, float* partial, int* nblk_out, int dtype, hipStream_t st) {
    BIU_DISPATCH_DTYPE(dtype, {
        constexpr int PE = 16 / sizeof(T);
        VPlan p = vplan(nvox(y), y->c, PE);
        VStats<T> f{dact(y)};
        hipLaunchKernelGGL((k_chan_reduce2_vec<VStats<T>, PE>), dim3(p.nblk), dim3(TPB), p.smem, st, f, nvox(y), y->c, p.ppv, p.vpb, partial);
        *nblk_out = p.nblk;
    });
    BIU_CHECK_LAUNCH("bn_stats_vec");
    return BIU_OK;
}
int biu_bn_bwd_reduce_vec(const biu_act* da, const biu_act* y, const float* scale, const float* shift, const float* slope,
                          const float* mean, const float* invstd, float* partial, int* nblk_out, int dtype, hipStream_t st) {
    BIU_DISPATCH_DTYPE(dtype, {
        constexpr int PE = 16 / sizeof(T);
        VPlan p = vplan(nvox(y), y->c, PE);
        VBnBwd<T> f{dact(da), dact(y), scale, shift, slope, mean, invstd};
        hipLaunchKernelGGL((k_chan_reduce2_vec<VBnBwd<T>, PE>), dim3(p.nblk), dim3(TPB), p.smem, st, f, nvox(y), y->c, p.ppv, p.vpb, partial);
        *nblk_out = p.nblk;
    });
    BIU_CHECK_LAUNCH("bn_bwd_reduce_vec");
    return BIU_OK;
}

__global__ void k_partial_sum0(const float* __restrict__ partial, int nblk, int C, float* __restrict__ out) {
    __shared__ double red[TPB];
    const int c = blockIdx.x;
    double a = 0;
    for (int b = threadIdx.x; b < nblk; b += TPB) a += partial[((i64)b * C + c) * 2];
    red[threadIdx.x] = a;
    __syncthreads();
    for (int s = TPB / 2; s > 0; s >>= 1) {
        if (threadIdx.x < s) red[threadIdx.x] += red[threadIdx.x + s];
        __syncthreads();
    }
    if (threadIdx.x == 0) out[c] = (float)red[0];
}
size_t biu_chan_sum_workspace(int c) { return (size_t)BIU_BN_MAX_PARTIALS * c * 2 * sizeof(float); }
int biu_chan_sum_vec(const biu_act* a, float* out, void* ws, int dtype, hipStream_t st) {
    int nblk = 0;
    BIU_DISPATCH_DTYPE(dtype, {
        constexpr int PE = 16 / sizeof(T);
        VPlan p = vplan(nvox(a), a->c, PE);
        VSum<T> f{dact(a)};
        hipLaunchKernelGGL((k_chan_reduce2_vec<VSum<T>, PE>), dim3(p.nblk), dim3(TPB), p.smem, st, f, nvox(a), a->c, p.ppv, p.vpb, (float*)ws);
        nblk = p.nblk;
    });
    BIU_CHECK_LAUNCH("chan_sum_vec");
    hipLaunchKernelGGL(k_partial_sum0, dim3(a->c), dim3(TPB), 0, st, (const float*)ws, nblk, a->c, out);
    BIU_CHECK_LAUNCH("partial_sum0");
    return BIU_OK;
}

template <typename T, int C, int O, bool RED>
__global__ __launch_bounds__(TPB) void k_head_bwd_fused(DAct x, DXf xf, const float* __restrict__ w, int cout,
                                                        const float* __restrict__ dl, DAct dx, int want_dx,
                                                        float* __restrict__ partial ,
                                                        const float* __restrict__ mean, const float* __restrict__ invstd,
                                                        float* __restrict__ bn_partial) {
    constexpr int G = 16 / sizeof(T);
    __shared__ float wsm[O * C];
    __shared__ float xsc[C], xsh[C], xsl[C];
    __shared__ float red[4][O * C + O];
    for (int i = threadIdx.x; i < O * C; i += TPB) wsm[i] = (i / C) < cout ? w[i] : 0.f;
    for (int i = threadIdx.x; i < C; i += TPB) {
        xsc[i] = xf.scale ? xf.scale[i] : 1.f;
        xsh[i] = xf.shift ? xf.shift[i] : 0.f;
        xsl[i] = xf.slope ? xf.slope[i] : 1.f;
    }
    __syncthreads();
    const i64 S = (i64)x.d * x.h * x.w;
    const i64 total = (i64)x.n * S;
    float aw[O][C], ab[O];
    float r1[RED ? C : 1], r2[RED ? C : 1];
#pragma unroll
    for (int o = 0; o < O; ++o) {
        ab[o] = 0.f;
#pragma unroll
        for (int c = 0; c < C; ++c) aw[o][c] = 0.f;
    }
    if (RED) {
#pragma unroll
        for (int c = 0; c < C; ++c) r1[c] = r2[c] = 0.f;
    }
    for (i64 v = (i64)blockIdx.x * TPB + threadIdx.x; v < total; v += (i64)gridDim.x * TPB) {
        const i64 n = v / S, s = v % S;
        float g[O];
#pragma unroll
        for (int o = 0; o < O; ++o) {
            g[o] = (o < cout) ? dl[(n * cout + o) * S + s] : 0.f;
            ab[o] += g[o];
        }
        const T* src = (const T*)x.p + v * x.pitch;
        T* dst = want_dx ? (T*)dx.p + v * dx.pitch : nullptr;
#pragma unroll
        for (int c0 = 0; c0 < C; c0 += G) {
            Pack<T, G> in = *(const Pack<T, G>*)(src + c0);
            Pack<T, G> od;
#pragma unroll
            for (int j = 0; j < G; ++j) {
                const int c = c0 + j;
                float t = fmaf(xsc[c], to_f(in.v[j]), xsh[c]);
                t = t > 0.f ? t : xsl[c] * t;
                float d = 0.f;
#pragma unroll
                for (int o = 0; o < O; ++o) {
                    aw[o][c] = fmaf(g[o], t, aw[o][c]);
                    d = fmaf(g[o], wsm[o * C + c], d);
                }
                od.v[j] = from_f<T>(d);
                if (RED) {
                    const float yv = to_f(in.v[j]);
                    const float dz = to_f(od.v[j]) * (fmaf(xsc[c], yv, xsh[c]) > 0.f ? 1.f : xsl[c]);
                    r1[c] += dz;
                    r2[c] = fmaf(dz, yv, r2[c]);
                }
            }
            if (want_dx) *(Pack<T, G>*)(dst + c0) = od;
        }
    }
    const int lane = threadIdx.x & 63, wave = threadIdx.x >> 6;
#pragma unroll
    for (int o = 0; o < O; ++o) {
#pragma unroll
        for (int c = 0; c < C; ++c) {
            const float r = wave_sum(aw[o][c]);
            if (lane == 0) red[wave][o * C + c] = r;
        }
        const float rb = wave_sum(ab[o]);
        if (lane == 0) red[wave][O * C + o] = rb;
    }
    __syncthreads();
    for (int i = threadIdx.x; i < O * C + O; i += TPB)
        partial[(i64)blockIdx.x * (O * C + O) + i] = red[0][i] + red[1][i] + red[2][i] + red[3][i];
    if (RED) {
        __shared__ float redb[4][2 * C];
#pragma unroll
        for (int c = 0; c < C; ++c) {
            const float a1 = wave_sum(r1[c]), a2 = wave_sum(r2[c]);
            if (lane == 0) { redb[wave][2 * c] = a1; redb[wave][2 * c + 1] = a2; }
        }
        __syncthreads();
        for (int c = threadIdx.x; c < C; c += TPB) {
            const float s1v = redb[0][2 * c] + redb[1][2 * c] + redb[2][2 * c] + redb[3][2 * c];
            const float s2v = redb[0][2 * c + 1] + redb[1][2 * c + 1] + redb[2][2 * c + 1] + redb[3][2 * c + 1];
            bn_partial[((i64)blockIdx.x * C + c) * 2 + 0] = s1v;
            bn_partial[((i64)blockIdx.x * C + c) * 2 + 1] = invstd[c] * (s2v - mean[c] * s1v);
        }
    }
}

__global__ void k_head_bwd_finalize(const float* __restrict__ partial, int nblk, int C, int O, int cout, float* dw, float* db) {
    __shared__ double red[TPB];
    const int i = blockIdx.x;
    double a = 0;
    for (int b = threadIdx.x; b < nblk; b += TPB) a += partial[(i64)b * (O * C + O) + i];
    red[threadIdx.x] = a;
    __syncthreads();
    for (int s = TPB / 2; s > 0; s >>= 1) {
        if (threadIdx.x < s) red[threadIdx.x] += red[threadIdx.x + s];
        __syncthreads();
    }
    if (threadIdx.x == 0) {
        if (i < O * C) {
            const int o = i / C, c = i % C;
            if (o < cout && dw) dw[o * C + c] = (float)red[0];
        } else {
            const int o = i - O * C;
            if (o < cout && db) db[o] = (float)red[0];
        }
    }
}

#define HEAD_FUSED_BLOCKS 1024
bool biu_head_bwd_fused_ok(const biu_act* x, const biu_act* dx, int cout, int dtype) {
    const int c = x->c;
    if (!(c == 8 || c == 16 || c == 32 || c == 64)) return false;
    if (cout < 1 || cout > 4 || c * (cout == 3 ? 4 : cout) > 128) return false;
    const int g = 16 / (int)dsize(dtype);
    if (!vec_ok(x, g, dtype)) return false;
    if (dx && !vec_ok(dx, g, dtype)) return false;
    return true;
}
size_t biu_head_bwd_fused_workspace(int cin) { return (size_t)HEAD_FUSED_BLOCKS * (4 * cin + 4) * sizeof(float); }

template <typename T, int C>
static int head_fused_t(const biu_act* x, const biu_xform* xf, const float* w, int cout, const float* dl, const biu_act* dx, float* dw,
                        float* db, void* ws, hipStream_t st, const float* mean = nullptr, const float* invstd = nullptr,
                        float* bn_partial = nullptr, int* bn_nblk = nullptr) {
    const i64 total = nvox(x);
    int nblk = (int)((total + TPB * 8 - 1) / (TPB * 8));
    if (nblk > HEAD_FUSED_BLOCKS) nblk = HEAD_FUSED_BLOCKS;
    if (nblk < 1) nblk = 1;
    DAct dxa = dx ? dact(dx) : dact(x);
    const int O = cout == 3 ? 4 : cout;
    if (bn_partial) {
        if constexpr (C <= 32) {
            if (O == 2) hipLaunchKernelGGL((k_head_bwd_fused<T, C, 2, true>), dim3(nblk), dim3(TPB), 0, st, dact(x), dxf(xf), w, cout, dl, dxa, 1, (float*)ws, mean, invstd, bn_partial);
            else hipLaunchKernelGGL((k_head_bwd_fused<T, C, 1, true>), dim3(nblk), dim3(TPB), 0, st, dact(x), dxf(xf), w, cout, dl, dxa, 1, (float*)ws, mean, invstd, bn_partial);
            *bn_nblk = nblk;
        }
    } else {
        if constexpr (C <= 32) {
            if (O == 4) hipLaunchKernelGGL((k_head_bwd_fused<T, C, 4, false>), dim3(nblk), dim3(TPB), 0, st, dact(x), dxf(xf), w, cout, dl, dxa, dx ? 1 : 0, (float*)ws, nullptr, nullptr, nullptr);
        }
        if (O == 2) hipLaunchKernelGGL((k_head_bwd_fused<T, C, 2, false>), dim3(nblk), dim3(TPB), 0, st, dact(x), dxf(xf), w, cout, dl, dxa, dx ? 1 : 0, (float*)ws, nullptr, nullptr, nullptr);
        if (O == 1) hipLaunchKernelGGL((k_head_bwd_fused<T, C, 1, false>), dim3(nblk), dim3(TPB), 0, st, dact(x), dxf(xf), w, cout, dl, dxa, dx ? 1 : 0, (float*)ws, nullptr, nullptr, nullptr);
    }
    BIU_CHECK_LAUNCH("head_bwd_fused");
    hipLaunchKernelGGL(k_head_bwd_finalize, dim3(O * C + O), dim3(TPB), 0, st, (const float*)ws, nblk, C, O, cout, dw, db);
    BIU_CHECK_LAUNCH("head_bwd_finalize");
    return BIU_OK;
}
bool biu_head_bwd_bnred_ok(const biu_act* x, const biu_act* dx, int cout, int dtype) {
    return dx && x->c <= 32 && cout <= 2 && biu_head_bwd_fused_ok(x, dx, cout, dtype);
}
int biu_head_bwd_bnred_fused(const biu_act* x, const biu_xform* xf, const float* w, int cout, const float* dl, const biu_act* dx, float* dw,
                             float* db, void* ws, const float* mean, const float* invstd, float* bn_partial, int* bn_nblk, int dtype,
                             hipStream_t st) {
    BIU_DISPATCH_DTYPE(dtype, {
        switch (x->c) {
            case 8: return head_fused_t<T, 8>(x, xf, w, cout, dl, dx, dw, db, ws, st, mean, invstd, bn_partial, bn_nblk);
            case 16: return head_fused_t<T, 16>(x, xf, w, cout, dl, dx, dw, db, ws, st, mean, invstd, bn_partial, bn_nblk);
            default: return head_fused_t<T, 32>(x, xf, w, cout, dl, dx, dw, db, ws, st, mean, invstd, bn_partial, bn_nblk);
        }
    });
    return BIU_OK;
}
int biu_head_bwd_fused(const biu_act* x, const biu_xform* xf, const float* w, int cout, const float* dl, const biu_act* dx, float* dw,
                       float* db, void* ws, size_t ws_bytes, int dtype, hipStream_t st) {
    BIU_REQUIRE(ws && ws_bytes >= biu_head_bwd_fused_workspace(x->c), BIU_ERR_WORKSPACE, "head_bwd: workspace too small");
    BIU_DISPATCH_DTYPE(dtype, {
        switch (x->c) {
            case 8: return head_fused_t<T, 8>(x, xf, w, cout, dl, dx, dw, db, ws, st);
            case 16: return head_fused_t<T, 16>(x, xf, w, cout, dl, dx, dw, db, ws, st);
            case 32: return head_fused_t<T, 32>(x, xf, w, cout, dl, dx, dw, db, ws, st);
            default: return head_fused_t<T, 64>(x, xf, w, cout, dl, dx, dw, db, ws, st);
        }
    });
    return BIU_OK;
}

struct RowPlan { int cg, rows, grid; };
static RowPlan row_plan(i64 total_vox, int C, int PE) {
    RowPlan p;
    p.cg = C / PE;
    p.rows = TPB / p.cg;
    i64 want = (total_vox + (i64)p.rows * 8 - 1) / ((i64)p.rows * 8);
    if (want < 1) want = 1;
    if (want > 4096) want = 4096;
    p.grid = (int)want;
    return p;
}
bool biu_rowvec_ok(const biu_act* a, int dtype) {
    const int pe = 16 / (int)dsize(dtype);
    return a->c % pe == 0 && a->c / pe <= TPB && vec_ok(a, pe, dtype);
}

template <typename T>
__global__ __launch_bounds__(TPB) void k_bn_bwd_apply_rv(DAct da, DAct y, const float* __restrict__ scale, const float* __restrict__ shift,
                                                         const float* __restrict__ slope, const float* __restrict__ A,
                                                         const float* __restrict__ B, const float* __restrict__ Cc, DAct dy, int cg, int rows) {
    constexpr int PE = 16 / sizeof(T);
    const int g = threadIdx.x % cg, row = threadIdx.x / cg;
    if (row >= rows) return;
    const int c0 = g * PE;
    float sc[PE], sh[PE], sl[PE], ka[PE], kb[PE], kc[PE];
#pragma unroll
// ... 517 lines not shown
```

bio_image_unet_amd/engine.py:

```python
from __future__ import annotations

import ctypes as C
import os
import weakref
from typing import Dict, List, Optional, Sequence, Tuple

import torch
from torch import nn

from . import _lib
from ._lib import BIU_BF16, BIU_F32, BN_MAX_PARTIALS, biu_act, biu_xform, check, lib

LRELU_SLOPE = 0.1


def _stream():
    return C.c_void_p(torch.cuda.current_stream().cuda_stream)


def _ptr(t: Optional[torch.Tensor]):
    return C.c_void_p(t.data_ptr()) if t is not None else None


def _disabled(token: str, env: Optional[str] = None) -> bool:
    return token in (os.environ.get("BIU_DISABLE", "") if env is None else env).split(",")


_NO_CAPTURE_FORK = _disabled("capturefork")
_NO_SIDE_CHAIN = _disabled("sidechain")
_NO_PREPACK = _disabled("prepack")
_SIDE_WGRAD_VOX = int(os.environ.get("BIU_SIDE_WGRAD_VOX", str(4 * 32 ** 3)))

class Buf:

    def __init__(self, eng: "Engine", n, d, h, w, c):
        self.eng = eng
        self.shape = (n, d, h, w, c)
        self.t = torch.empty(self.shape, dtype=eng.tdtype, device=eng.device)
        self.g: Optional[torch.Tensor] = None
        self.scale = torch.ones(c, dtype=torch.float32, device=eng.device)
        self.shift = torch.zeros(c, dtype=torch.float32, device=eng.device)
        self.slope = torch.ones(c, dtype=torch.float32, device=eng.device)
        self.leaves: Dict[Tuple[int, int], bool] = {}
        self.lazy: Dict[Tuple[int, int], bool] = {}
        self.ncons: Dict[Tuple[int, int], int] = {}
        self.nwr: Dict[Tuple[int, int], int] = {}
        self.producer: Dict[Tuple[int, int], "Node"] = {}
        self.acts = []

    def slice(self, c0: int, c: int, lazy: bool) -> "Act":
        self.leaves[(c0, c)] = False
        self.lazy[(c0, c)] = lazy
        return Act(self, c0, c, [(c0, c)])

    def span(self, c0: int, c: int) -> "Act":
        keys = sorted(k for k in self.leaves if c0 <= k[0] < c0 + c)
        cov = c0
        for k0, kc in keys:
            assert k0 == cov, "span has a hole"
            cov += kc
        assert cov == c0 + c, "span does not end on a slice boundary"
        return Act(self, c0, c, keys)

    def full(self) -> "Act":
        keys = sorted(self.leaves)
        cov = 0
        for c0, c in keys:
            assert c0 == cov, "concat buffer has a hole"
            cov += c
        assert cov == self.shape[4]
        return Act(self, 0, cov, keys)

    def grad(self) -> torch.Tensor:
        assert self.t is not None, "a released buffer has no gradient either"
        if self.g is None:
            self.g = torch.empty(self.shape, dtype=self.eng.tdtype, device=self.eng.device)
        return self.g

    def release(self):
        self.t = None
        self.g = None
        for a in self.acts:
            a._a.p = None
# ... 112 lines not shown
class CatBuf:

    def __init__(self, eng: "Engine", space, c_first, c_second):
        n, d, h, w = space
        self.c_first, self.c_second = c_first, c_second
        self.bufs = (eng.new_buf(n, d, h, w, c_first), eng.new_buf(n, d, h, w, c_second))
        self.acts = [None, None]

    def slice(self, c0: int, c: int, lazy: bool) -> Act:
        k = 0 if (c0, c) == (0, self.c_first) else 1
        assert (c0, c) == ((0, self.c_first) if k == 0 else (self.c_first, self.c_second)), "a planar concat has exactly two slices"
        self.acts[k] = self.bufs[k].slice(0, c, lazy)
        return self.acts[k]

    def full(self) -> CatAct:
        assert self.acts[0] is not None and self.acts[1] is not None, "both parts must be produced before the concatenation is read"
        return CatAct(self.acts[0], self.acts[1])


class Node:
    params: Sequence[nn.Parameter] = ()
    label = "node"

    def fwd(self, eng: "Engine"):
        raise NotImplementedError

    def bwd(self, eng: "Engine"):
        raise NotImplementedError


def _ksize(w: torch.Tensor):
    if w.dim() == 5:
        return tuple(w.shape[2:])
    return (1,) + tuple(w.shape[2:])


class ConvBlockNode(Node):

    def __init__(self, eng, seq: nn.Sequential, xin: Act, yout: Act, dropout_follows: bool = False, fold_src: Optional[Act] = None,
                 convt: Optional["ConvTNode"] = None):
        conv, bn = seq[0], seq[1]
        self.conv, self.bn, self.xin, self.y = conv, bn, xin, yout
        self.fold_src, self.fold_slot, self.fold_dg_slot, self.fold_wg, self.fold_all = None, None, None, False, False
        self.foldt, self.foldt_blob, self.foldt_ver = None, None, None
        self.fold_ws, self.fold_ev = None, None
        self.wg_ws, self.wg_ev = None, None
        act = seq[2] if len(seq) > 2 else None
        self.slope = float(act.negative_slope) if isinstance(act, nn.LeakyReLU) else (0.0 if isinstance(act, nn.ReLU) else 1.0)
        xin.consumed()
        if len(yout.leaves) == 1:
            yout.buf.producer[yout.leaves[0]] = self
        self.red_partial: Optional[torch.Tensor] = None
        self.red_nblk = 0
        self.kd, self.kh, self.kw = _ksize(conv.weight)
        self.dil = int(conv.dilation[0])
        drop = seq[3] if len(seq) > 3 else None
        if drop is not None and getattr(drop, "p", 0.0) != 0.0 and not dropout_follows:
            raise NotImplementedError("Dropout p != 0 needs a DropoutNode behind the block (models.Unet_v0 / BabyUnet build one)")
        assert tuple(conv.weight.shape[:2]) == (yout.c, xin.c), (conv.weight.shape, yout.c, xin.c)
        assert xin.space == yout.space
        self.params = [conv.weight, conv.bias, bn.weight, bn.bias]
        cout = yout.c
        dev = eng.device
        self.save_mean = torch.empty(cout, dtype=torch.float32, device=dev)
        self.save_invstd = torch.empty(cout, dtype=torch.float32, device=dev)
        yout.vec("slope").fill_(self.slope)
        eng.need_partial(cout)
        eng.need_partial_floats(lib.biu_conv_fwd_stats_floats(yout.a(), self.kd))
        if (convt is not None and isinstance(xin, CatAct) and len(xin.parts) == 2 and xin.parts[0] is convt.y and convt.kd == 2
                and (self.kd, self.kh, self.kw, self.dil) == (3, 3, 3, 1) and convt.up.bias is not None
                and lib.biu_foldt_ok(convt.xin.a(), xin.parts[1].a(), yout.a(), eng.dtype)
                and lib.biu_foldt_bwd_weight_workspace(convt.xin.c, xin.parts[1].c, cout, eng.dtype) > 0):
            self.foldt = convt
            lo, skip = convt.xin, xin.parts[1]
            self.foldt_blob = torch.empty(lib.biu_foldt_packed_bytes(lo.c, skip.c, cout, eng.dtype), dtype=torch.uint8, device=dev)
            eng.need_partial_floats(lib.biu_foldt_fwd_stats_floats(lo.a(), yout.a()))
            eng.need_ws(lib.biu_foldt_bwd_weight_workspace(lo.c, skip.c, cout, eng.dtype))
            self.params = [conv.weight, conv.bias, bn.weight, bn.bias]
        if (fold_src is not None and (self.kd, self.kh, self.kw, self.dil) == (3, 3, 3, 1) and not isinstance(xin, CatAct)
                and fold_src.c == xin.c and lib.biu_upconv_ok(fold_src.a(), yout.a(), eng.dtype)):
            self.fold_src = fold_src
            self.fold_slot = {"buf": torch.empty(lib.biu_upconv_packed_bytes(0, xin.c, cout, eng.dtype), dtype=torch.uint8, device=dev), "ver": None}
            nb1 = lib.biu_upconv_packed_bytes(1, xin.c, cout, eng.dtype)
            if nb1:
                self.fold_dg_slot = {"buf": torch.empty(nb1, dtype=torch.uint8, device=dev), "ver": None}
            wsf = lib.biu_upconv_bwd_weight_workspace(xin.c, cout, eng.dtype)
            if wsf:
                self.fold_wg = True
                eng.need_ws(wsf)
            self.fold_all = self.fold_dg_slot is not None and self.fold_wg
            eng.need_partial_floats(lib.biu_upconv_fwd_stats_floats(fold_src.a(), yout.a()))
        self.pk_f = eng.packed_slot(0, xin.c, cout, self.kd, self.kh, self.kw, self.dil)
        self.pk_b = eng.packed_slot(1, xin.c, cout, self.kd, self.kh, self.kw, self.dil)
        self.ws_bytes = lib.biu_conv_bwd_weight_workspace(xin.c, cout, self.kd, self.kh, self.kw, eng.dtype)
        eng.need_ws(self.ws_bytes)
        eng.need_ws(lib.biu_conv_split_workspace(xin.c, yout.a(), None, self.kd, self.kh, self.kw, self.dil, eng.dtype))
        if isinstance(xin, CatAct):
            eng.need_ws(lib.biu_conv_split_workspace(cout, xin.parts[0].a(), xin.parts[1].a(), self.kd, self.kh, self.kw, self.dil, eng.dtype))
        else:
            eng.need_ws(lib.biu_conv_split_workspace(cout, xin.a(), None, self.kd, self.kh, self.kw, self.dil, eng.dtype))

    def fwd(self, eng):
        st = _stream()
        w, b = self.conv.weight.data, self.conv.bias.data if self.conv.bias is not None else None
        packed = eng.pack(self.pk_f, 0, self.conv.weight, self.xin.c, self.y.c, self.kd, self.kh, self.kw)
        bn = self.bn
# ... 95 lines not shown

    def _bwd_foldt(self, eng, st, scale, shift, slope, A, B, Cc, dw, dy_sum=None):
        ct, skip, y = self.foldt, self.xin.parts[1], self.y
        lo = ct.xin
        dwt, dbt = eng.new_grad(ct.up.weight), eng.new_grad(ct.up.bias)
        side = eng.chain_stream()
        if side is None:
            check(lib.biu_foldt_bwd_weight_bn(lo.a(), lo.xf(), skip.a(), skip.xf(), y.g(), y.a(), scale, shift, slope, _ptr(A), _ptr(B), _ptr(Cc), _ptr(dy_sum),
                                              _ptr(self.conv.weight.data), _ptr(ct.up.weight.data), _ptr(ct.up.bias.data), ct.y.c, _ptr(dw), _ptr(dwt),
                                              _ptr(dbt), _ptr(eng.ws), eng.ws_bytes, eng.dtype, st), "foldt_bwd_weight_bn")
            eng.add_grad(ct.up.weight, dwt)
            eng.add_grad(ct.up.bias, dbt)
            deferred = False
        else:
            if self.fold_ws is None:
                self.fold_ws = torch.empty(lib.biu_foldt_bwd_weight_workspace(lo.c, skip.c, y.c, eng.dtype), dtype=torch.uint8, device=eng.device)
                self.fold_ev = (torch.cuda.Event(), torch.cuda.Event())
            args = (lo.a(), lo.xf(), skip.a(), skip.xf(), y.g(), y.a(), scale, shift, slope, _ptr(A), _ptr(B), _ptr(Cc), _ptr(dy_sum),
                    _ptr(self.conv.weight.data), _ptr(ct.up.weight.data), _ptr(ct.up.bias.data), ct.y.c, _ptr(dw), _ptr(dwt), _ptr(dbt),
                    _ptr(self.fold_ws), self.fold_ws.numel(), eng.dtype)
            check(lib.biu_foldt_bwd_weight_bn_phase(*args, 1 | 4, st), "foldt_bwd_weight_bn_phase(1 | 4)")
            cur = torch.cuda.current_stream()
            ready, done = self.fold_ev
            ready.record(cur)
            side.wait_event(ready)
            label = lib.label
            with torch.cuda.stream(side):
                lib.label = label + "/chain"
                check(lib.biu_foldt_bwd_weight_bn_phase(*args, 2, _stream()), "foldt_bwd_weight_bn_phase(2)")
                done.record(side)
            lib.label = label
            eng.defer_grads(done, [(ct.up.weight, dwt), (ct.up.bias, dbt), (self.conv.weight, dw)], keep=(A, B, Cc, dy_sum))
            deferred = True
        blob = self._foldt_packed(st)
        want_lo = eng.wants_grad(lo)
        up = _fusable_producer(lo) if want_lo else None
        if not want_lo:
            raise NotImplementedError("foldt: the coarse input of a decoder level always wants its gradient")
        if up is not None:
            need = lib.biu_foldt_bwd_data_bnred_floats(lo.a())
            if up.red_partial is None or up.red_partial.numel() < need:
                up.red_partial = torch.empty(need, dtype=torch.float32, device=eng.device)
            n_up = C.c_int(0)
            check(lib.biu_foldt_bwd_data(y.g(), blob, lo.g(), 0, skip.g(), int(skip.g_written()), lo.a(), *up.red_coeffs(), _ptr(up.red_partial),
                                         up.red_partial.numel(), C.byref(n_up), _ptr(eng.ws), eng.ws_bytes, eng.dtype, st), "foldt_bwd_data")
            up.red_nblk = n_up.value
        else:
            check(lib.biu_foldt_bwd_data(y.g(), blob, lo.g(), int(lo.g_written()), skip.g(), int(skip.g_written()), None, None, None, None, None, None,
                                         None, 0, None, _ptr(eng.ws), eng.ws_bytes, eng.dtype, st), "foldt_bwd_data")
        lo.mark_g()
        skip.mark_g()
        return deferred

    def bwd(self, eng):
        if not self.y.g_written():
            return
        st = _stream()
        y, cout = self.y, self.y.c
        scale, shift, slope = _ptr(y.vec("scale")), _ptr(y.vec("shift")), _ptr(y.vec("slope"))
        nblk = C.c_int(0)
        if self.red_nblk:
            partial, nblk.value, self.red_nblk = self.red_partial, self.red_nblk, 0
        else:
            partial = eng.partial
            check(lib.biu_bn_bwd_reduce(y.g(), y.a(), scale, shift, slope, _ptr(self.save_mean), _ptr(self.save_invstd),
                                        _ptr(partial), C.byref(nblk), eng.dtype, st), "bn_bwd_reduce")
        dgamma, dbeta = eng.new_grad(self.bn.weight), eng.new_grad(self.bn.bias)
        A, B, Cc = eng.coef[0][:cout], eng.coef[1][:cout], eng.coef[2][:cout]
        dw = eng.new_grad(self.conv.weight)
        dy_sum = None
        if self.batch_stats:
            check(lib.biu_bn_bwd_finalize(_ptr(partial), nblk.value, cout, float(y.nvox), scale, _ptr(self.save_mean),
                                          _ptr(self.save_invstd), _ptr(dgamma), _ptr(dbeta), _ptr(A), _ptr(B), _ptr(Cc), st),
                  "bn_bwd_finalize")
            db = eng.zero_like_bias(self.conv.bias) if self.conv.bias is not None else None
        else:
            dy_sum = torch.empty(cout, dtype=torch.float32, device=eng.device)
            check(lib.biu_bn_bwd_finalize_eval(_ptr(partial), nblk.value, cout, scale, _ptr(dgamma), _ptr(dbeta), _ptr(dy_sum), _ptr(A), _ptr(B),
                                               _ptr(Cc), st), "bn_bwd_finalize_eval")
            db = dy_sum if self.conv.bias is not None else None
        cat = self.xin.parts if isinstance(self.xin, CatAct) else None
        if self.foldt is not None:
            if not self._bwd_foldt(eng, st, scale, shift, slope, A, B, Cc, dw, dy_sum):
                eng.add_grad(self.conv.weight, dw)
            if db is not None:
                eng.add_grad(self.conv.bias, db)
            eng.add_grad(self.bn.weight, dgamma)
            eng.add_grad(self.bn.bias, dbeta)
            return
        if cat:
            check(lib.biu_conv_bwd_weight_cat(cat[0].a(), cat[0].xf(), cat[1].a(), cat[1].xf(), y.g(), y.a(), scale, shift, slope,
                                              _ptr(A), _ptr(B), _ptr(Cc), self.kd, self.kh, self.kw, self.dil, _ptr(dw), _ptr(eng.ws),
                                              eng.ws_bytes, eng.dtype, st), "conv_bwd_weight_cat")
        elif self.fold_wg:
            check(lib.biu_upconv_bwd_weight_bn(self.fold_src.a(), self.fold_src.xf(), y.g(), y.a(), scale, shift, slope, _ptr(A), _ptr(B),
                                               _ptr(Cc), _ptr(dw), _ptr(eng.ws), eng.ws_bytes, eng.dtype, st), "upconv_bwd_weight_bn")
        elif self.kd == 3 and eng.tdtype == torch.bfloat16 and y.nvox <= _SIDE_WGRAD_VOX and eng.chain_stream() is not None:
            side = eng.chain_stream()
            check(lib.biu_bn_bwd_apply(y.g(), y.a(), scale, shift, slope, _ptr(A), _ptr(B), _ptr(Cc), y.g(), eng.dtype, st), "bn_bwd_apply")
            if self.wg_ws is None:
                self.wg_ws = torch.empty(max(lib.biu_conv_bwd_weight_workspace(self.xin.c, cout, self.kd, self.kh, self.kw, eng.dtype), 16), dtype=torch.uint8,
                                         device=eng.device)
                self.wg_ev = (torch.cuda.Event(), torch.cuda.Event())
            ready, done = self.wg_ev
            ready.record(torch.cuda.current_stream())
            side.wait_event(ready)
            label = lib.label
            with torch.cuda.stream(side):
                lib.label = label + "/wgrad"
                check(lib.biu_conv_bwd_weight(self.xin.a(), self.xin.xf(), y.g(), self.kd, self.kh, self.kw, self.dil, _ptr(dw), None, _ptr(self.wg_ws),
                                              self.wg_ws.numel(), eng.dtype, _stream()), "conv_bwd_weight")
                done.record(side)
            lib.label = label
            eng.defer_grads(done, [(self.conv.weight, dw)])
            dw = None
        else:
            check(lib.biu_conv_bwd_weight_bn(self.xin.a(), self.xin.xf(), y.g(), y.a(), scale, shift, slope, _ptr(A), _ptr(B),
                                             _ptr(Cc), self.kd, self.kh, self.kw, self.dil, _ptr(dw), _ptr(eng.ws), eng.ws_bytes,
                                             eng.dtype, st), "conv_bwd_weight_bn")
        if dw is not None:
            eng.add_grad(self.conv.weight, dw)
        if db is not None:
            eng.add_grad(self.conv.bias, db)
        eng.add_grad(self.bn.weight, dgamma)
        eng.add_grad(self.bn.bias, dbeta)
        if cat:
            packed = eng.pack(self.pk_b, 1, self.conv.weight, self.xin.c, cout, self.kd, self.kh, self.kw)
            check(lib.biu_conv_bwd_data_cat(y.g(), _ptr(self.conv.weight.data), packed, self.kd, self.kh, self.kw, self.dil,
                                            cat[0].g(), cat[0].g_accumulate(), cat[1].g(), cat[1].g_accumulate(), _ptr(eng.ws), eng.ws_bytes, eng.dtype, st),
                  "conv_bwd_data_cat")
            cat[0].mark_g()
            cat[1].mark_g()
        elif self.fold_dg_slot is not None and eng.wants_grad(self.fold_src):
            ver = (self.conv.weight.data_ptr(), self.conv.weight._version)
            if self.fold_dg_slot["ver"] != ver:
                check(lib.biu_upconv_pack(1, _ptr(self.conv.weight.data), self.xin.c, cout, eng.dtype, _ptr(self.fold_dg_slot["buf"]), st), "upconv_pack")
                self.fold_dg_slot["ver"] = ver
            check(lib.biu_upconv_bwd_data(y.g(), _ptr(self.fold_dg_slot["buf"]), self.fold_src.g(), int(self.fold_src.g_written()), eng.dtype, st),
                  "upconv_bwd_data")
            self.fold_src.mark_g()
        elif eng.wants_grad(self.xin):
            packed = eng.pack(self.pk_b, 1, self.conv.weight, self.xin.c, cout, self.kd, self.kh, self.kw)
            up = _fusable_producer(self.xin)
            if up is not None:
                part = up.red_buffer(eng, self.kd, 0)
                n_up = C.c_int(0)
                check(lib.biu_conv_bwd_data_bnred(y.g(), _ptr(self.conv.weight.data), packed, self.kd, self.kh, self.kw,
                                                  self.dil, self.xin.g(), self.xin.a(), *up.red_coeffs(), _ptr(part),
                                                  part.numel(), C.byref(n_up), _ptr(eng.ws), eng.ws_bytes, eng.dtype, st), "conv_bwd_data_bnred")
                up.red_nblk = n_up.value
            else:
                check(lib.biu_conv_bwd_data(y.g(), _ptr(self.conv.weight.data), packed, self.kd, self.kh, self.kw, self.dil,
                                            self.xin.g(), int(self.xin.g_written()), _ptr(eng.ws), eng.ws_bytes, eng.dtype, st), "conv_bwd_data")
            self.xin.mark_g()

    def red_buffer(self, eng, kd, transposed) -> torch.Tensor:
        need = lib.biu_bwd_data_bnred_floats(self.y.a(), kd, transposed)
        if self.red_partial is None or self.red_partial.numel() < need:
            self.red_partial = torch.empty(need, dtype=torch.float32, device=eng.device)
        return self.red_partial

    def red_coeffs(self):
        y = self.y
        return (_ptr(y.vec("scale")), _ptr(y.vec("shift")), _ptr(y.vec("slope")), _ptr(self.save_mean),
                _ptr(self.save_invstd))


def _fusable_producer(xin: Act):
# ... 236 lines not shown
        check(lib.biu_gate_bwd(self.e_.a(), self.e_.xf(), self.psi_.a(), self.psi_.xf(), self.y.g(), self.e_.g(),
                               int(self.e_.g_written()), self.psi_.g(), eng.dtype, _stream()), "gate_bwd")
        self.e_.mark_g()
        self.psi_.mark_g()


_ACT_CODE = {None: 0, "none": 0, "sigmoid": 1, "tanh": 2, "relu": 3}


class HeadNode(Node):

    def __init__(self, eng, conv: nn.Module, xin: Act, activation, want_logits: bool, want_act: bool):
        self.conv, self.xin = conv, xin
        xin.consumed()
        self.cout = conv.weight.shape[0]
        assert conv.weight.shape[1] == xin.c
        if activation not in _ACT_CODE:
            activation = None
        self.activation = activation
        self.act = _ACT_CODE[activation]
        self.want_logits, self.want_act = want_logits, want_act
        self.params = [conv.weight, conv.bias]
        eng.need_ws(lib.biu_head_bwd_workspace(xin.c))
        self.logits = self.activated = None

    def out_shape(self, eng):
        x = self.xin
        return (x.n, self.cout, x.d, x.h, x.w) if eng.nd == 3 else (x.n, self.cout, x.h, x.w)

    def fwd(self, eng):
        shp = self.out_shape(eng)
        self.logits = torch.empty(shp, dtype=torch.float32, device=eng.device) if self.want_logits else None
        self.activated = torch.empty(shp, dtype=torch.float32, device=eng.device) if self.want_act else None
        w = self.conv.weight.data.reshape(self.cout, self.xin.c)
        check(lib.biu_head_fwd(self.xin.a(), self.xin.xf(), _ptr(w), _ptr(self.conv.bias.data), self.cout, self.act,
                               _ptr(self.logits), _ptr(self.activated), eng.dtype, _stream()), "head_fwd")

    def dlogits(self, eng, g_logits, g_act, a, dst=None, ctot=None, c0=0):
        if g_act is None and dst is None and g_logits.dtype == torch.float32 and g_logits.is_contiguous():
            return g_logits
        shp = self.out_shape(eng)
        n, spatial = shp[0], 1
        for v in shp[2:]:
            spatial *= v
        if dst is None:
            dst, ctot, c0 = torch.empty(shp, dtype=torch.float32, device=eng.device), self.cout, 0
        f32 = lambda t: None if t is None else t.contiguous().float()
        gl, ga = f32(g_logits), f32(g_act)
        self._keep = (gl, ga, a)
        check(lib.biu_head_dlogits(_ptr(gl), _ptr(ga), _ptr(a) if ga is not None else None, self.act, n, self.cout, spatial,
                                   _ptr(dst), ctot, c0, _stream()), "head_dlogits")
        return dst

    def bwd_with(self, eng, dl: Optional[torch.Tensor]):
        if dl is None:
            return
        dl = dl.contiguous().float()
        st = _stream()
        dw, db = eng.new_grad(self.conv.weight), eng.new_grad(self.conv.bias)
        want_dx = eng.wants_grad(self.xin)
        assert not self.xin.g_written(), "heads that share a trunk go through Engine._backward_heads"
        up = self.xin.last_writer_producer() if (want_dx and self.xin.xf() is not None) else None
        if up is not None:
            part = up.red_buffer(eng, up.kd, 0)
            n_up = C.c_int(0)
            check(lib.biu_head_bwd_bnred(self.xin.a(), self.xin.xf(), _ptr(self.conv.weight.data), self.cout, _ptr(dl),
                                         self.xin.g(), _ptr(dw), _ptr(db), _ptr(eng.ws), eng.ws_bytes, _ptr(up.save_mean),
                                         _ptr(up.save_invstd), _ptr(part), part.numel(), C.byref(n_up), eng.dtype, st),
                  "head_bwd_bnred")
            up.red_nblk = n_up.value
        else:
            check(lib.biu_head_bwd(self.xin.a(), self.xin.xf(), _ptr(self.conv.weight.data), self.cout, _ptr(dl),
                                   self.xin.g() if want_dx else None, _ptr(dw), _ptr(db), _ptr(eng.ws), eng.ws_bytes,
                                   eng.dtype, st), "head_bwd")
        eng.add_grad(self.conv.weight, dw)
        eng.add_grad(self.conv.bias, db)
        if want_dx:
            self.xin.mark_g()


class Engine:

    def __init__(self, device, tdtype, nd: int):
        if torch.device(device).type != "cuda":
            raise RuntimeError("bio_image_unet_amd executes only through its HIP kernels on an MI355X; "
                               f"got device '{device}'. There is no CPU fallback.")
        self.device, self.tdtype, self.nd = torch.device(device), tdtype, nd
        self.dtype = {torch.float32: BIU_F32, torch.bfloat16: BIU_BF16}[tdtype]
        self.nodes: List[Node] = []
        self.heads: List[HeadNode] = []
        self.bufs: List[Buf] = []
        self.inputs: List[Act] = []
        self._partial_c = 0
        self.ws_bytes = 0
        self.partial = self.ws = None
        self.coef = None
        self.grads: Dict[nn.Parameter, torch.Tensor] = {}
        self.nbt_bump: List[torch.Tensor] = []
        self.grad_mode = False
        self.module_training = True
        self.input_requires_grad = False
        self._packed: Dict[int, dict] = {}
        self._zero_flat, self._zero_used = None, 0
        self._slots: List[dict] = []
        self._job_key, self._job_tab = None, None
        self.grad_hook = None
        self.grad_alloc = None
        self.trace = None
        self.generation = 0
        self._live = None
        self._side = None
        self._deferred = []
        self._fold_ev = None

    def busy(self) -> bool:
        return self._live is not None and self._live() is not None

    def invalidate_packed(self):
        for s in self._slots:
            s["ver"] = None
# ... 214 lines not shown
        return self._side

    def defer_grads(self, done: "torch.cuda.Event", grads, keep=()):
        self._deferred.append((done, grads, keep))

    def _flush_deferred(self, keep_last: int):
        while len(self._deferred) > keep_last:
            done, grads, _ = self._deferred.pop(0)
            torch.cuda.current_stream().wait_event(done)
            for p, g in grads:
                self.add_grad(p, g)

    def backward(self, head_grads: Sequence[Optional[torch.Tensor]]):
        self.grads = {}
        self._deferred = []
        self._pseen: Dict[nn.Parameter, int] = {}
        self._zero_flat, self._zero_used = None, 0
        for b in self.bufs:
            for k in b.leaves:
                b.leaves[k] = False
                b.nwr[k] = 0
        lib.label = "head:bwd"
        if self.trace:
            self.trace("bwd", ("heads", head_grads), "pre")
        self._backward_heads(head_grads)
        if self.trace:
            self.trace("bwd", ("heads", head_grads), "post")
        for nd_ in reversed(self.nodes):
            if isinstance(nd_, HeadNode):
                continue
            lib.label = nd_.label + ":bwd"
            if self.trace:
                self.trace("bwd", nd_, "pre")
            self._flush_deferred(2)
            nd_.bwd(self)
            if self.trace:
                self.trace("bwd", nd_, "post")
        self._flush_deferred(0)
        return self.grads

    def _backward_heads(self, head_grads):
        live = [(h, g) for h, g in zip(self.heads, head_grads) if g is not None]
        if not live:
            return
        groups: Dict[int, list] = {}
        for h, g in live:
            groups.setdefault(id(h.xin), []).append((h, g))
        for grp in groups.values():
            self._backward_head_group(grp)

    def _backward_head_group(self, live):
        if len(live) == 1:
            h, (gl, ga, a) = live[0]
            h.bwd_with(self, h.dlogits(self, gl, ga, a))
            return
        x = live[0][0].xin
        assert all(h.xin is x for h, _ in live)
        cout = sum(h.cout for h, _ in live)
        shp = live[0][0].out_shape(self)
        dl = torch.empty((shp[0], cout) + tuple(shp[2:]), dtype=torch.float32, device=self.device)
        key = tuple(id(h) for h, _ in live)
        if not hasattr(self, "_stack_w"):
            self._stack_w = {}
        if key not in self._stack_w:
            self._stack_w[key] = torch.empty((cout, x.c), dtype=torch.float32, device=self.device)
        w, o = self._stack_w[key], 0
        for h, (gl, ga, a) in live:
            w[o:o + h.cout].copy_(h.conv.weight.data.reshape(h.cout, x.c))
            h.dlogits(self, gl, ga, a, dst=dl, ctot=cout, c0=o)
            o += h.cout
        dw = torch.empty_like(w)
        db = torch.empty(cout, dtype=torch.float32, device=self.device)
        up = None
        if self.wants_grad(x) and x.xf() is not None and not x.g_written() and len(x.leaves) == 1:
            k = x.leaves[0]
            cand = x.buf.producer.get(k)
            if (x.buf.ncons.get(k, 0) == len(live) and cand is not None and getattr(cand, "batch_stats", False)
                    and cand.y.c == x.c and cand.y.c0 == x.c0):
                up = cand
        if up is not None:
            part = up.red_buffer(self, up.kd, 0)
            n_up = C.c_int(0)
            check(lib.biu_head_bwd_bnred(x.a(), x.xf(), _ptr(w), cout, _ptr(dl), x.g(), _ptr(dw), _ptr(db), _ptr(self.ws), self.ws_bytes,
                                         _ptr(up.save_mean), _ptr(up.save_invstd), _ptr(part), part.numel(), C.byref(n_up), self.dtype,
                                         _stream()), "head_bwd_bnred(stacked)")
            up.red_nblk = n_up.value
        else:
            check(lib.biu_head_bwd(x.a(), x.xf(), _ptr(w), cout, _ptr(dl), x.g(), _ptr(dw), _ptr(db), _ptr(self.ws),
                                   self.ws_bytes, self.dtype, _stream()), "head_bwd(stacked)")
        x.mark_g()
        o = 0
        for h, _ in live:
            self.add_grad(h.conv.weight, dw[o:o + h.cout].reshape(h.conv.weight.shape).clone())
            self.add_grad(h.conv.bias, db[o:o + h.cout].clone())
            o += h.cout

    def input_grads(self) -> List[Optional[torch.Tensor]]:
        outs = []
        st = _stream()
        for act in self.inputs:
            if not self.input_requires_grad or not act.g_written():
                outs.append(None)
                continue
            shp = (act.n, act.c, act.d, act.h, act.w) if self.nd == 3 else (act.n, act.c, act.h, act.w)
            t = torch.empty(shp, dtype=torch.float32, device=self.device)
            ga = biu_act(act.buf.grad().data_ptr(), act.n, act.d, act.h, act.w, act.c, act.buf.shape[4])
            check(lib.biu_to_nchw(C.byref(ga), None, _ptr(t), self.dtype, st), "to_nchw")
            outs.append(t)
        return outs


class _Token:
    __slots__ = ("__weakref__",)


class _NetFn(torch.autograd.Function):

    @staticmethod
    def forward(ctx, eng: Engine, n_inputs: int, out_spec, *tensors):
        xs, ctx.n_inputs = tensors[:n_inputs], n_inputs
        if eng.busy():
            raise RuntimeError("engine re-entered while an earlier forward still awaits its backward (models take a second "
                               "engine for that case: this is a bug in the caller of engine.run)")
        eng.load_inputs(xs)
        eng.forward()
        ctx.eng, ctx.out_spec = eng, out_spec
        ctx.generation = eng.generation
        if eng.grad_mode:
            ctx.token = _Token()
            eng._live = weakref.ref(ctx.token)
        else:
            eng._live = None
        outs = []
        for hi, kind in out_spec:
            h = eng.heads[hi]
            outs.append(h.logits if kind == "logits" else h.activated)
        ctx.act_slot = {hi: i for i, (hi, kind) in enumerate(out_spec) if kind == "act"}
        ctx.save_for_backward(*[outs[i] for i in ctx.act_slot.values()])
        for h in eng.heads:
            h.logits = h.activated = None
        return tuple(outs)

    @staticmethod
    def backward(ctx, *gouts):
        eng: Engine = ctx.eng
        if ctx.generation != eng.generation:
            raise RuntimeError("backward of a forward whose activations were overwritten: the engine ran another forward of the "
                               "same input shape in between (generation %d, now %d)" % (ctx.generation, eng.generation))
        per_head: Dict[int, List[Optional[torch.Tensor]]] = {}
        for (hi, kind), g in zip(ctx.out_spec, gouts):
            slot = per_head.setdefault(hi, [None, None])
            slot[0 if kind == "logits" else 1] = g
        saved = dict(zip(ctx.act_slot.keys(), ctx.saved_tensors))
        head_grads = []
        for hi, h in enumerate(eng.heads):
            gl, ga = per_head.get(hi, [None, None])
            head_grads.append((gl, ga, saved.get(hi)) if (gl is not None or ga is not None) else None)
        grads = eng.backward(head_grads)
        dxs = eng.input_grads()
        pg = [grads.pop(p, None) for p in eng.params]
        eng.grads = {}
        del grads
        ctx.token = None
        eng._live = None
        eng.generation += 1
        return (None, None, None, *dxs, *pg)


def run(eng: Engine, xs: Sequence[torch.Tensor], out_spec):
    eng.grad_mode = torch.is_grad_enabled()
    eng.input_requires_grad = eng.grad_mode and any(x.requires_grad for x in xs)
    return _NetFn.apply(eng, len(xs), tuple(out_spec), *xs, *eng.params)
```

include/biu.h:

```cpp
#ifndef BIU_H
#define BIU_H

#include <stddef.h>
#include <stdint.h>

#ifdef __cplusplus
extern "C" {
#endif

typedef void* biu_stream;

enum { BIU_F32 = 0, BIU_BF16 = 1 };

typedef enum {
    BIU_OK = 0,
    BIU_ERR_SHAPE = -1,
    BIU_ERR_UNSUPPORTED = -2,
    BIU_ERR_ALIGN = -3,
    BIU_ERR_WORKSPACE = -4,
    BIU_ERR_LAUNCH = -5
} biu_status;

typedef struct {
    void*   p;
// ... 12 lines not shown
int  biu_version(void);

int  biu_set_fp32_products(int mode);

int  biu_set_fp32_products_3d(int mode);


size_t biu_conv_packed_bytes(int kind, int cin, int cout, int kd, int kh, int kw, int dilation, int dtype);
int    biu_conv_pack(int kind, const float* w, int cin, int cout, int kd, int kh, int kw, int dtype,
                     void* packed, biu_stream stream);

typedef struct biu_pack_job {
    const void* w;
    void* packed;
    int32_t transposed, kind, cin, cout, kd, kh, kw, reserved;
} biu_pack_job;
int biu_pack_batch(const biu_pack_job* jobs, int n, int dtype, biu_stream stream);

size_t biu_conv_split_workspace(int cin, const biu_act* y, const biu_act* y1, int kd, int kh, int kw, int dilation, int dtype);

int biu_conv_fwd(const biu_act* x, const biu_xform* xf, const float* w, const void* packed,
                 const float* bias, int kd, int kh, int kw, int dilation,
                 const biu_act* y, void* ws, size_t ws_bytes, int dtype, biu_stream stream);

size_t biu_conv_fwd_stats_floats(const biu_act* y, int kd);
int biu_conv_fwd_stats(const biu_act* x, const biu_xform* xf, const float* w, const void* packed,
                       const float* bias, int kd, int kh, int kw, int dilation, const biu_act* y,
                       float* bn_partial, size_t bn_partial_floats, int* bn_nblk, void* ws, size_t ws_bytes, int dtype,
                       biu_stream stream);

int biu_conv_bwd_data(const biu_act* dy, const float* w, const void* packed,
                      int kd, int kh, int kw, int dilation,
                      const biu_act* dx, int accumulate, void* ws, size_t ws_bytes, int dtype, biu_stream stream);

size_t biu_bwd_data_bnred_floats(const biu_act* dx, int kd, int transposed);
int biu_conv_bwd_data_bnred(const biu_act* dy, const float* w, const void* packed, int kd, int kh, int kw, int dilation,
                            const biu_act* dx, const biu_act* y_up, const float* scale, const float* shift,
                            const float* slope, const float* mean, const float* invstd, float* partial,
                            size_t partial_floats, int* nblk, void* ws, size_t ws_bytes, int dtype, biu_stream stream);
int biu_convt_bwd_data_bnred(const biu_act* dy, const float* w, const void* packed, int kd, const biu_act* dx,
                             const biu_act* y_up, const float* scale, const float* shift, const float* slope,
                             const float* mean, const float* invstd, float* partial, size_t partial_floats, int* nblk,
                             int dtype, biu_stream stream);

size_t biu_conv_bwd_weight_workspace(int cin, int cout, int kd, int kh, int kw, int dtype);
int biu_conv_bwd_weight(const biu_act* x, const biu_xform* xf, const biu_act* dy,
                        int kd, int kh, int kw, int dilation,
                        float* dw, float* dbias, void* ws, size_t ws_bytes, int dtype, biu_stream stream);

int biu_conv_bwd_weight_bn(const biu_act* x, const biu_xform* xf, const biu_act* da, const biu_act* y,
                           const float* scale, const float* shift, const float* slope, const float* coefA,
                           const float* coefB, const float* coefC, int kd, int kh, int kw, int dilation,
                           float* dw, void* ws, size_t ws_bytes, int dtype, biu_stream stream);

#define BIU_BN_MAX_PARTIALS 1024
int biu_bn_stats(const biu_act* y, float* partial, int* nblk_out, int dtype, biu_stream stream);

int biu_bn_finalize(const float* partial, int nblk, int c, double count,
                    const float* gamma, const float* beta, float* running_mean, float* running_var,
                    float momentum, float eps, float* scale, float* shift,
                    float* save_mean, float* save_invstd, biu_stream stream);

int biu_bn_eval_affine(int c, const float* gamma, const float* beta, const float* running_mean,
                       const float* running_var, float eps, float* scale, float* shift, biu_stream stream);

int biu_xform_apply(const biu_act* x, const biu_xform* xf, const biu_act* out, int dtype, biu_stream stream);

int biu_bn_bwd_reduce(const biu_act* da, const biu_act* y, const float* scale, const float* shift,
                      const float* slope, const float* save_mean, const float* save_invstd,
                      float* partial, int* nblk_out, int dtype, biu_stream stream);
int biu_bn_bwd_finalize(const float* partial, int nblk, int c, double count,
                        const float* scale, const float* save_mean, const float* save_invstd,
                        float* dgamma, float* dbeta, float* coefA, float* coefB, float* coefC,
                        biu_stream stream);
int biu_bn_bwd_finalize_eval(const float* partial, int nblk, int c, const float* scale,
                             float* dgamma, float* dbeta, float* dbias, float* coefA, float* coefB, float* coefC,
                             biu_stream stream);
int biu_bn_bwd_apply(const biu_act* da, const biu_act* y, const float* scale, const float* shift,
                     const float* slope, const float* coefA, const float* coefB, const float* coefC,
                     const biu_act* dy, int dtype, biu_stream stream);

int biu_maxpool_fwd(const biu_act* x, const biu_xform* xf, const biu_act* out, int dtype, biu_stream stream);
int biu_maxpool_bwd(const biu_act* x, const biu_xform* xf, const biu_act* dout, const biu_act* dx,
                    int accumulate, int dtype, biu_stream stream);
int biu_maxpool_bwd_bnred(const biu_act* x, const biu_xform* xf, const biu_act* dout, const biu_act* dx, int accumulate,
                          const float* mean, const float* invstd, float* partial, size_t partial_floats, int* nblk,
                          int dtype, biu_stream stream);
int biu_nearest_down_fwd(const biu_act* x, const biu_xform* xf, const biu_act* out, int dtype, biu_stream stream);
int biu_nearest_down_bwd(const biu_act* dout, const biu_act* dx, int accumulate, int dtype, biu_stream stream);
int biu_nearest_up_fwd(const biu_act* x, const biu_xform* xf, const biu_act* out, int dtype, biu_stream stream);
int biu_nearest_up_bwd(const biu_act* dout, const biu_act* dx, int accumulate, int dtype, biu_stream stream);

int    biu_upconv_ok(const biu_act* x, const biu_act* y, int dtype);
size_t biu_upconv_packed_bytes(int kind, int cin, int cout, int dtype);
int    biu_upconv_pack(int kind, const float* w, int cin, int cout, int dtype, void* packed, biu_stream stream);
int    biu_upconv_bwd_data(const biu_act* dy, const void* packed, const biu_act* dx, int accumulate, int dtype, biu_stream stream);
size_t biu_upconv_bwd_weight_workspace(int cin, int cout, int dtype);
int    biu_upconv_bwd_weight_bn(const biu_act* x, const biu_xform* xf, const biu_act* da, const biu_act* y, const float* scale,
                                const float* shift, const float* slope, const float* coefA, const float* coefB, const float* coefC,
                                float* dw, void* ws, size_t ws_bytes, int dtype, biu_stream stream);
size_t biu_upconv_fwd_stats_floats(const biu_act* x, const biu_act* y);
int    biu_upconv_fwd(const biu_act* x, const biu_xform* xf, const void* packed, const float* bias, const biu_act* y,
                      float* bn_partial, size_t bn_partial_floats, int* bn_nblk, int dtype, biu_stream stream);

int biu_bce_dice_blocks(long long per_sample);
int biu_bce_dice_fwd(const float* logits, const float* target, int n, long long per_sample, float* partial, biu_stream stream);
// ... 194 lines not shown
```

Before: 735.2 million voxels/s.

## Recompute head input gradient as rank-one product inside fused wgrad loader

```diff
diff --git a/bio_image_unet_amd/_lib.py b/bio_image_unet_amd/_lib.py
--- a/bio_image_unet_amd/_lib.py
+++ b/bio_image_unet_amd/_lib.py
@@ -74,6 +74,8 @@
     "biu_conv_bwd_weight_workspace": (_Z, [_I, _I, _I, _I, _I, _I]),
     "biu_conv_bwd_weight": (_I, [_A, _X, _A, _I, _I, _I, _I, _P, _P, _P, _Z, _I, _P]),
     "biu_conv_bwd_weight_bn": (_I, [_A, _X, _A, _A, _P, _P, _P, _P, _P, _P, _I, _I, _I, _I, _P, _P, _Z, _I, _P]),
+    "biu_conv_bwd_weight_bn_rank1_ok": (_I, [_A, _A, _A, _I, _I, _I, _I, _I, _I]),
+    "biu_conv_bwd_weight_bn_rank1": (_I, [_A, _X, _P, _P, _I, _A, _A, _P, _P, _P, _P, _P, _P, _I, _I, _I, _I, _P, _P, _Z, _I, _P]),
     "biu_bn_stats": (_I, [_A, _P, C.POINTER(C.c_int), _I, _P]),
     "biu_bn_finalize": (_I, [_P, _I, _I, _D, _P, _P, _P, _P, _F, _F, _P, _P, _P, _P, _P]),
     "biu_bn_eval_affine": (_I, [_I, _P, _P, _P, _P, _F, _P, _P, _P]),
diff --git a/bio_image_unet_amd/csrc/biu_api.hip b/bio_image_unet_amd/csrc/biu_api.hip
--- a/bio_image_unet_amd/csrc/biu_api.hip
+++ b/bio_image_unet_amd/csrc/biu_api.hip
@@ -8,7 +8,7 @@
     "conv_fwd", "conv_dgrad", "conv_wgrad", "convt_fwd", "convt_dgrad", "convt_wgrad", "convt_all", "c1", "c1_mfma", "cat",
     "fused_stats", "wgrad_bn", "dgrad_bnred", "pool_pair", "pool_pipe", "pool_bnred", "head_bnred", "ksplit", "m16", "m16x2", "rr16",
     "wroll", "wroll16", "wroll2d", "upconv", "foldt", "foldall", "foldck8", "foldgemm", "croll", "froll", "prepack", "wsplitbn",
-    "capturefork", "sidechain",
+    "capturefork", "sidechain", "headrank1",
 };
 constexpr int kNumOffTokens = sizeof(kOffTokens) / sizeof(kOffTokens[0]);
 static_assert(kNumOffTokens <= 64, "BiuEnv::off holds one bit per token");
@@ -307,6 +307,29 @@
     int rc = biu_bn_bwd_apply(da, y, scale, shift, slope, coefA, coefB, coefC, da, dtype, stream);
     if (rc != BIU_OK) return rc;
     return biu_conv_bwd_weight(x, xf, da, kd, kh, kw, dilation, dw, nullptr, ws, ws_bytes, dtype, stream);
+}
+
+static bool rank1_y_ok(const biu_act* y, int dtype) {
+    const size_t es = dsize(dtype);
+    return ((uintptr_t)y->p % 16) == 0 && ((size_t)y->pitch * es) % 16 == 0 && (i64)y->d * y->h * y->w * y->pitch * (i64)es < (1LL << 32) - 65536;
+}
+extern "C" int biu_conv_bwd_weight_bn_rank1_ok(const biu_act* x, const biu_act* dy, const biu_act* y, int head_cout, int kd, int kh, int kw,
+                                               int dilation, int dtype) {
+    if (!x || !dy || !y || !conv_args_ok(x, dy, kd, kh, kw, dilation) || !valid_act(y) || !same_space(y, dy) || y->c != dy->c) return 0;
+    if (head_cout != 1 || biu_off("conv_wgrad") || biu_off("wgrad_bn") || !rank1_y_ok(y, dtype)) return 0;
+    return biu_mfma_wgrad_rank1_ok(x, dy, kd, kh, kw, dilation, dtype) ? 1 : 0;
+}
+extern "C" int biu_conv_bwd_weight_bn_rank1(const biu_act* x, const biu_xform* xf, const float* dlogits, const float* w_head, int head_cout,
+                                            const biu_act* dy, const biu_act* y, const float* scale, const float* shift, const float* slope,
+                                            const float* coefA, const float* coefB, const float* coefC, int kd, int kh, int kw, int dilation,
+                                            float* dw, void* ws, size_t ws_bytes, int dtype, biu_stream stream) {
+    BIU_REQUIRE(biu_conv_bwd_weight_bn_rank1_ok(x, dy, y, head_cout, kd, kh, kw, dilation, dtype), BIU_ERR_UNSUPPORTED,
+                "conv_bwd_weight_bn_rank1: shapes not served by the rank-one loader (ask biu_conv_bwd_weight_bn_rank1_ok)");
+    BIU_REQUIRE(dlogits && w_head && dw && scale && shift && coefA && coefB && coefC, BIU_ERR_SHAPE, "conv_bwd_weight_bn_rank1: null pointer");
+    BIU_REQUIRE(ws && ws_bytes >= biu_mfma_wgrad_workspace(x->c, dy->c, kd, kh, kw, dtype), BIU_ERR_WORKSPACE,
+                "conv_bwd_weight_bn_rank1: workspace too small");
+    BnBwdFuse bn{y, scale, shift, slope, coefA, coefB, coefC, dlogits, w_head};
+    return biu_mfma_wgrad(x, xf, dy, kd, kh, kw, dw, nullptr, ws, ws_bytes, dtype, (hipStream_t)stream, &bn);
 }
 
 extern "C" int biu_conv_cat_ok(const biu_act* x0, const biu_act* x1, const biu_act* y, int kd, int kh, int kw, int dilation, int dtype) {
diff --git a/bio_image_unet_amd/csrc/biu_conv_mfma.hip b/bio_image_unet_amd/csrc/biu_conv_mfma.hip
--- a/bio_image_unet_amd/csrc/biu_conv_mfma.hip
+++ b/bio_image_unet_amd/csrc/biu_conv_mfma.hip
@@ -2338,6 +2338,7 @@
     int ypitch;
     const float* bn_scale; const float* bn_shift; const float* bn_slope;
     const float* bn_cA; const float* bn_cB; const float* bn_cC;
+    const float* r1_dl = nullptr; const float* r1_w = nullptr;
     float* dbias_out;
     int fold_par;
     size_t fold_slice_f;
@@ -3035,14 +3036,15 @@
 constexpr int WR_AB = WR_BV * WR_RS;
 constexpr int WR_NAI = WR_AB / 1024;
 constexpr int WR_NABUF = 3;
-constexpr size_t WR_LDS = (size_t)WR_NPAIR * WR_PAIRB + WR_NABUF * WR_AB + 9 * 32 * sizeof(float);
+constexpr size_t WR_LDS = (size_t)WR_NPAIR * WR_PAIRB + WR_NABUF * WR_AB + 10 * 32 * sizeof(float);
 
 __device__ __forceinline__ unsigned opaque_s(unsigned x) { asm volatile("" : "+s"(x)); return x; }
 template <int N> __device__ __forceinline__ void wait_vmcnt() { asm volatile("s_waitcnt vmcnt(%0)" ::"n"(N) : "memory"); }
 
-template <bool BNF, bool K2D, bool A16 = false>
+template <bool BNF, bool K2D, bool A16 = false, bool R1 = false>
 __global__ __launch_bounds__(512, 2) void k_wgrad_roll(WgradArgs a) {
     static_assert(!(K2D && A16), "the 16-channel plain operand form exists for volumes only");
+    static_assert(!R1 || (BNF && A16), "the rank-one loader belongs to the fused 16-channel form");
     using T = bf16_t;
     using F = Frag<T>;
     constexpr int TD = WR_TD, TH = WR_TH, TW = WR_TW, HW = WR_HW, PL = WR_PL, RS = WR_RS, PLB = WR_PLB, PAIRB = WR_PAIRB;
@@ -3054,7 +3056,7 @@
     char* bring = (char*)lds;
     char* abuf = bring + WR_NPAIR * PAIRB;
     float* lxf = (float*)(abuf + WR_NABUF * WR_AB);
-    constexpr int LB = 0, LBN = 3 * CT;
+    constexpr int LB = 0, LBN = 3 * CT, LR1 = 9 * CT;
 
     const int tid = threadIdx.x, lane = tid & 63;
     const int wave = __builtin_amdgcn_readfirstlane(tid >> 6);
@@ -3091,6 +3093,9 @@
         lxf[LB + 2 * CT + tid] = (b_xf && cb < a.CB) ? bl_[cbl] : 1.f;
     }
 
+    if constexpr (R1) {
+        if (tid < CT) lxf[LR1 + tid] = (it * CT + tid < a.CA) ? a.r1_w[it * CT + tid] : 0.f;
+    }
     floatx16 acc[NACC];
 #pragma unroll
     for (int t = 0; t < NACC; ++t)
@@ -3129,12 +3134,12 @@
 
     int cn = 0, ch0 = 0, cw0 = 0;
     v4u_t rsB, rsA;
-    __amdgpu_buffer_rsrc_t rsAr, rsYr;
+    __amdgpu_buffer_rsrc_t rsAr, rsYr, rsLr;
     struct Slot { unsigned bmask, amask; uint4 pa[BNF ? NAK : 1], pyv[BNF ? NAK : 1]; };
     Slot sl0, sl1;
     sl0.bmask = sl0.amask = sl1.bmask = sl1.amask = 0;
-    unsigned bbase[NBK], abase_[NAK], ybase_[BNF ? NAK : 1];
-    unsigned planeB = 0, planeA = 0, planeY = 0;
+    unsigned bbase[NBK], abase_[NAK], ybase_[BNF ? NAK : 1], lbase_[R1 ? NAK : 1];
+    unsigned planeB = 0, planeA = 0, planeY = 0, planeL = 0;
     auto set_column = [&](int col) __attribute__((always_inline)) {
         int c = col;
         const int wb_ = c % a.nbw; c /= a.nbw;
@@ -3146,6 +3151,11 @@
         rsAr = __builtin_amdgcn_make_buffer_rsrc((void*)(a.pa + (size_t)cn * sampA), 0, (int)(unsigned)sampA, 0x00020000);
         rsYr = __builtin_amdgcn_make_buffer_rsrc((void*)(a.py + (size_t)cn * sampY), 0, bn_fused ? (int)(unsigned)sampY : 0, 0x00020000);
         planeB = (unsigned)(a.BH * a.BW) * rowB; planeA = (unsigned)(a.GH * a.GW) * rowA; planeY = (unsigned)(a.GH * a.GW) * rowY;
+        if constexpr (R1) {
+            const size_t sampL = (size_t)a.GD * a.GH * a.GW * 4;
+            rsLr = __builtin_amdgcn_make_buffer_rsrc((void*)((const char*)a.r1_dl + (size_t)cn * sampL), 0, (int)(unsigned)sampL, 0x00020000);
+            planeL = (unsigned)(a.GH * a.GW) * 4u;
+        }
 #pragma unroll
         for (int k = 0; k < NBK; ++k) {
             const unsigned x = bco[k];
@@ -3161,9 +3171,10 @@
             const unsigned vox = (unsigned)(gh * a.GW + gw);
             abase_[k] = ok ? vox * rowA + (unsigned)ac0 * 2u + (x & 1023u) * planeA : 0xffffffffu;
             if constexpr (BNF) ybase_[k] = ok ? vox * rowY + (unsigned)ac0 * 2u + (x & 1023u) * planeY : 0xffffffffu;
+            if constexpr (R1) lbase_[k] = ok ? vox * 4u + (x & 1023u) * planeL : 0xffffffffu;
         }
     };
-    struct FetchCtx { int pair, buf; bool bd0, bd1, ad0, ad1; unsigned dofB, dofA, dofY; };
+    struct FetchCtx { int pair, buf; bool bd0, bd1, ad0, ad1; unsigned dofB, dofA, dofY, dofL; };
     auto fetch_ctx = [&](int pair, int gp0, int buf, int d0) __attribute__((always_inline)) -> FetchCtx {
         FetchCtx f;
         f.pair = pair; f.buf = buf;
@@ -3171,6 +3182,7 @@
         f.ad0 = d0 < a.GD; f.ad1 = d0 + 1 < a.GD;
         f.dofB = opaque_s((unsigned)gp0 * planeB);
         f.dofA = opaque_s((unsigned)d0 * planeA); f.dofY = opaque_s((unsigned)d0 * planeY);
+        if constexpr (R1) f.dofL = opaque_s((unsigned)d0 * planeL); else f.dofL = 0;
         f.pair = (int)opaque_s((unsigned)pair); f.buf = (int)opaque_s((unsigned)buf);
         return f;
     };
@@ -3184,9 +3196,13 @@
             const int k = i - NBK;
             const bool ok = abase_[k] != 0xffffffffu && ((aco[k] & 1u) ? f.ad1 : f.ad0);
             if constexpr (BNF) {
-                const auto v0 = __builtin_amdgcn_raw_buffer_load_b128(rsAr, ok ? (int)(abase_[k] + f.dofA) : -1, 0, 0);
+                if constexpr (R1) {
+                    sl.pa[k].x = __builtin_amdgcn_raw_buffer_load_b32(rsLr, ok ? (int)(lbase_[k] + f.dofL) : -1, 0, 0);
+                } else {
+                    const auto v0 = __builtin_amdgcn_raw_buffer_load_b128(rsAr, ok ? (int)(abase_[k] + f.dofA) : -1, 0, 0);
+                    sl.pa[k] = make_uint4(v0[0], v0[1], v0[2], v0[3]);
+                }
                 const auto v1 = __builtin_amdgcn_raw_buffer_load_b128(rsYr, ok ? (int)(ybase_[k] + f.dofY) : -1, 0, 0);
-                sl.pa[k] = make_uint4(v0[0], v0[1], v0[2], v0[3]);
                 sl.pyv[k] = make_uint4(v1[0], v1[1], v1[2], v1[3]);
             } else {
                 bload_lds16(ok ? abase_[k] + f.dofA : 0xffffffffu, rsA, lds0 + (unsigned)(WR_NPAIR * PAIRB + f.buf * WR_AB + (wave + 8 * k) * 1024));
@@ -3224,7 +3240,13 @@
                 for (int k = 0; k < NAK; ++k) {
                     if ((sl.amask >> k) & 1u) {
                         float g[PE], yy[PE];
-                        F::unpack(sl.pa[k], g);
+                        if constexpr (R1) {
+                            const float dlv = __uint_as_float(sl.pa[k].x);
+#pragma unroll
+                            for (int e = 0; e < PE; ++e) g[e] = (float)(T)fmaf(dlv, lxf[LR1 + apc * PE + e], 0.f);
+                        } else {
+                            F::unpack(sl.pa[k], g);
+                        }
                         F::unpack(sl.pyv[k], yy);
 #pragma unroll
                         for (int e = 0; e < PE; ++e) g[e] *= (fmaf(ks[e], yy[e], kh[e]) > 0.f ? 1.f : kl[e]);
@@ -3472,6 +3494,7 @@
 static int launch_wgrad_roll(WgradArgs a, hipStream_t st, bool k2d = false) {
     if (k2d) { a.GD = a.BD = a.N; a.N = 1; }
     const bool a16 = !k2d && a.CA == 16 && !biu_off("wroll16");
+    if (a.r1_dl && !(a16 && a.py)) return biu_fail(BIU_ERR_UNSUPPORTED, "wgrad_roll: the rank-one loader exists for the fused 16-channel form only");
     a.nbd = 1;
     a.nbh = (a.GH + WR_TH - 1) / WR_TH;
     a.nbw = (a.GW + WR_TW - 1) / WR_TW;
@@ -3492,7 +3515,8 @@
             hipFuncSetAttribute((const void*)k_wgrad_roll<false, true>, hipFuncAttributeMaxDynamicSharedMemorySize, (int)WR_LDS) != hipSuccess ||
             hipFuncSetAttribute((const void*)k_wgrad_roll<true, true>, hipFuncAttributeMaxDynamicSharedMemorySize, (int)WR_LDS) != hipSuccess ||
             hipFuncSetAttribute((const void*)k_wgrad_roll<false, false, true>, hipFuncAttributeMaxDynamicSharedMemorySize, (int)WR_LDS) != hipSuccess ||
-            hipFuncSetAttribute((const void*)k_wgrad_roll<true, false, true>, hipFuncAttributeMaxDynamicSharedMemorySize, (int)WR_LDS) != hipSuccess)
+            hipFuncSetAttribute((const void*)k_wgrad_roll<true, false, true>, hipFuncAttributeMaxDynamicSharedMemorySize, (int)WR_LDS) != hipSuccess ||
+            hipFuncSetAttribute((const void*)k_wgrad_roll<true, false, true, true>, hipFuncAttributeMaxDynamicSharedMemorySize, (int)WR_LDS) != hipSuccess)
             return biu_fail(BIU_ERR_LAUNCH, "wgrad_roll: cannot reserve %zu bytes of LDS", WR_LDS);
         attr_set = true;
     }
@@ -3509,7 +3533,8 @@
             if (with_bn) hipLaunchKernelGGL((k_wgrad_roll<true, true>), dim3(g, pairs), dim3(512), WR_LDS, st, b);
             else hipLaunchKernelGGL((k_wgrad_roll<false, true>), dim3(g, pairs), dim3(512), WR_LDS, st, b);
         } else if (a16) {
-            if (with_bn) hipLaunchKernelGGL((k_wgrad_roll<true, false, true>), dim3(g, pairs), dim3(512), WR_LDS, st, b);
+            if (with_bn && b.r1_dl) hipLaunchKernelGGL((k_wgrad_roll<true, false, true, true>), dim3(g, pairs), dim3(512), WR_LDS, st, b);
+            else if (with_bn) hipLaunchKernelGGL((k_wgrad_roll<true, false, true>), dim3(g, pairs), dim3(512), WR_LDS, st, b);
             else hipLaunchKernelGGL((k_wgrad_roll<false, false, true>), dim3(g, pairs), dim3(512), WR_LDS, st, b);
         } else {
             if (with_bn) hipLaunchKernelGGL((k_wgrad_roll<true, false>), dim3(g, pairs), dim3(512), WR_LDS, st, b);
@@ -3641,6 +3666,16 @@
     return BIU_OK;
 }
 
+bool biu_mfma_wgrad_rank1_ok(const biu_act* x, const biu_act* dy, int kd, int kh, int kw, int dilation, int dtype) {
+    if (dtype != BIU_BF16 || kd != 3 || dy->c != 16 || !biu_mfma_wgrad_ok(x, dy, kd, kh, kw, dilation, dtype)) return false;
+    if (biu_off("wroll") || biu_off("wroll16") || (x->c == 16 && !biu_off("rr16"))) return false;
+    if (!biu_off("wsplitbn") && x->c > 32 && nvox(dy) <= 4 * 32 * 32 * 32) return false;
+    if ((i64)x->d * x->h * x->w * 4 >= (1LL << 32)) return false;
+    WgradArgs a;
+    a.N = x->n; a.GD = x->d; a.GH = x->h; a.GW = x->w;
+    return biu_env().roll_always || wroll_fits(a);
+}
+
 int biu_mfma_wgrad(const biu_act* x, const biu_xform* xf, const biu_act* dy, int kd, int kh, int kw, float* dw, float* dbias,
                    void* ws, size_t ws_bytes, int dtype, hipStream_t st, const BnBwdFuse* bn, const biu_act* x1, const biu_xform* xf1,
                    int dw_ld_cols, int dw_c_off) {
@@ -3655,6 +3690,7 @@
         a.py = (const char*)bn->y->p; a.ypitch = bn->y->pitch;
         a.bn_scale = bn->scale; a.bn_shift = bn->shift; a.bn_slope = bn->slope;
         a.bn_cA = bn->cA; a.bn_cB = bn->cB; a.bn_cC = bn->cC;
+        a.r1_dl = bn->r1_dl; a.r1_w = bn->r1_w;
     } else {
         a.py = nullptr; a.ypitch = 0;
         a.bn_scale = a.bn_shift = a.bn_slope = a.bn_cA = a.bn_cB = a.bn_cC = nullptr;
@@ -3679,7 +3715,8 @@
     const size_t need = wgrad_acc_bytes(a.CA, a.CB, taps);
     BIU_REQUIRE(ws_bytes >= need + (dbias ? biu_chan_sum_workspace(dy->c) : 0), BIU_ERR_WORKSPACE, "wgrad_mfma: workspace %zu too small", ws_bytes);
     if (int zr = zero_ws(ws, need, nullptr, 0, st)) return zr;
-    if (dtype == BIU_BF16 && kd == 3 && a.CB == 16 && !x1 && !biu_off("rr16")) rc = launch_wgrad<bf16_t, 3, 3, 1, 4, 8, 16, 1, 1, true>(a, st);
+    if (a.r1_dl) rc = launch_wgrad_roll(a, st);
+    else if (dtype == BIU_BF16 && kd == 3 && a.CB == 16 && !x1 && !biu_off("rr16")) rc = launch_wgrad<bf16_t, 3, 3, 1, 4, 8, 16, 1, 1, true>(a, st);
     else if (dtype == BIU_BF16 && kd == 3 && !biu_off("wroll") && wroll_fits(a)) rc = launch_wgrad_roll(a, st);
     else if (dtype == BIU_BF16 && kd == 1 && !biu_off("wroll") && !biu_off("wroll2d") &&
              wroll2d_fits(a, (i64)nvox(dy) * dy->pitch * 2, (i64)nvox(x) * x->pitch * 2 > (x1 ? (i64)nvox(x1) * x1->pitch * 2 : 0) ? (i64)nvox(x) * x->pitch * 2 : (i64)nvox(x1) * x1->pitch * 2,
diff --git a/bio_image_unet_amd/csrc/biu_direct.hip b/bio_image_unet_amd/csrc/biu_direct.hip
--- a/bio_image_unet_amd/csrc/biu_direct.hip
+++ b/bio_image_unet_amd/csrc/biu_direct.hip
@@ -1180,12 +1180,13 @@
                                   const biu_act* dx, float* dw, float* dbias, void* ws, size_t ws_bytes, const float* mean,
                                   const float* invstd, float* partial, size_t partial_floats, int* nblk, int dtype,
                                   biu_stream stream) {
-    BIU_REQUIRE(valid_act(x) && w && dlogits && dx && valid_act(dx) && same_space(x, dx) && dx->c == x->c && cout > 0 &&
+    BIU_REQUIRE(valid_act(x) && w && dlogits && (!dx || (valid_act(dx) && same_space(x, dx) && dx->c == x->c)) && cout > 0 &&
                     cout <= HEAD_MAX_COUT, BIU_ERR_SHAPE, "head_bwd_bnred: bad arguments");
     BIU_REQUIRE(xf && xf->scale && xf->shift && mean && invstd && partial && nblk, BIU_ERR_SHAPE, "head_bwd_bnred: null vector");
     BIU_REQUIRE(partial_floats >= (size_t)BIU_BN_MAX_PARTIALS * x->c * 2, BIU_ERR_WORKSPACE, "head_bwd_bnred: partial buffer too small");
     if (!biu_off("head_bnred") && biu_head_bwd_bnred_ok(x, dx, cout, dtype) && ws && ws_bytes >= biu_head_bwd_fused_workspace(x->c))
         return biu_head_bwd_bnred_fused(x, xf, w, cout, dlogits, dx, dw, dbias, ws, mean, invstd, partial, nblk, dtype, (hipStream_t)stream);
+    BIU_REQUIRE(dx, BIU_ERR_UNSUPPORTED, "head_bwd_bnred: dx = NULL needs the fused kernel (C <= 32, cout <= 2, 16-byte rows)");
     int rc = biu_head_bwd(x, xf, w, cout, dlogits, dx, dw, dbias, ws, ws_bytes, dtype, stream);
     if (rc != BIU_OK) return rc;
     return biu_bn_bwd_reduce(dx, x, xf->scale, xf->shift, xf->slope, mean, invstd, partial, nblk, dtype, stream);
diff --git a/bio_image_unet_amd/csrc/biu_internal.h b/bio_image_unet_amd/csrc/biu_internal.h
--- a/bio_image_unet_amd/csrc/biu_internal.h
+++ b/bio_image_unet_amd/csrc/biu_internal.h
@@ -72,7 +72,10 @@
 struct BnBwdFuse {
     const biu_act* y;
     const float *scale, *shift, *slope, *cA, *cB, *cC;
+    const float* r1_dl = nullptr;
+    const float* r1_w = nullptr;
 };
+bool biu_mfma_wgrad_rank1_ok(const biu_act* x, const biu_act* dy, int kd, int kh, int kw, int dilation, int dtype);
 int biu_mfma_wgrad(const biu_act* x, const biu_xform* xf, const biu_act* dy, int kd, int kh, int kw, float* dw,
                    float* dbias, void* ws, size_t ws_bytes, int dtype, hipStream_t st, const BnBwdFuse* bn = nullptr,
                    const biu_act* x1 = nullptr, const biu_xform* xf1 = nullptr, int dw_ld_cols = 0, int dw_c_off = 0);
diff --git a/bio_image_unet_amd/csrc/biu_special.hip b/bio_image_unet_amd/csrc/biu_special.hip
--- a/bio_image_unet_amd/csrc/biu_special.hip
+++ b/bio_image_unet_amd/csrc/biu_special.hip
@@ -505,7 +505,7 @@
     return BIU_OK;
 }
 
-template <typename T, int C, int O, bool RED>
+template <typename T, int C, int O, bool RED, bool STORE = true>
 __global__ __launch_bounds__(TPB) void k_head_bwd_fused(DAct x, DXf xf, const float* __restrict__ w, int cout,
                                                         const float* __restrict__ dl, DAct dx, int want_dx,
                                                         float* __restrict__ partial ,
@@ -545,7 +545,7 @@
             ab[o] += g[o];
         }
         const T* src = (const T*)x.p + v * x.pitch;
-        T* dst = want_dx ? (T*)dx.p + v * dx.pitch : nullptr;
+        T* dst = (STORE && want_dx) ? (T*)dx.p + v * dx.pitch : nullptr;
 #pragma unroll
         for (int c0 = 0; c0 < C; c0 += G) {
             Pack<T, G> in = *(const Pack<T, G>*)(src + c0);
@@ -569,7 +569,7 @@
                     r2[c] = fmaf(dz, yv, r2[c]);
                 }
             }
-            if (want_dx) *(Pack<T, G>*)(dst + c0) = od;
+            if (STORE && want_dx) *(Pack<T, G>*)(dst + c0) = od;
         }
     }
     const int lane = threadIdx.x & 63, wave = threadIdx.x >> 6;
@@ -649,7 +649,10 @@
     const int O = cout == 3 ? 4 : cout;
     if (bn_partial) {
         if constexpr (C <= 32) {
-            if (O == 2) hipLaunchKernelGGL((k_head_bwd_fused<T, C, 2, true>), dim3(nblk), dim3(TPB), 0, st, dact(x), dxf(xf), w, cout, dl, dxa, 1, (float*)ws, mean, invstd, bn_partial);
+            if (!dx) {
+                if (O == 2) hipLaunchKernelGGL((k_head_bwd_fused<T, C, 2, true, false>), dim3(nblk), dim3(TPB), 0, st, dact(x), dxf(xf), w, cout, dl, dxa, 0, (float*)ws, mean, invstd, bn_partial);
+                else hipLaunchKernelGGL((k_head_bwd_fused<T, C, 1, true, false>), dim3(nblk), dim3(TPB), 0, st, dact(x), dxf(xf), w, cout, dl, dxa, 0, (float*)ws, mean, invstd, bn_partial);
+            } else if (O == 2) hipLaunchKernelGGL((k_head_bwd_fused<T, C, 2, true>), dim3(nblk), dim3(TPB), 0, st, dact(x), dxf(xf), w, cout, dl, dxa, 1, (float*)ws, mean, invstd, bn_partial);
             else hipLaunchKernelGGL((k_head_bwd_fused<T, C, 1, true>), dim3(nblk), dim3(TPB), 0, st, dact(x), dxf(xf), w, cout, dl, dxa, 1, (float*)ws, mean, invstd, bn_partial);
             *bn_nblk = nblk;
         }
@@ -666,7 +669,7 @@
     return BIU_OK;
 }
 bool biu_head_bwd_bnred_ok(const biu_act* x, const biu_act* dx, int cout, int dtype) {
-    return dx && x->c <= 32 && cout <= 2 && biu_head_bwd_fused_ok(x, dx, cout, dtype);
+    return x->c <= 32 && cout <= 2 && biu_head_bwd_fused_ok(x, dx, cout, dtype);
 }
 int biu_head_bwd_bnred_fused(const biu_act* x, const biu_xform* xf, const float* w, int cout, const float* dl, const biu_act* dx, float* dw,
                              float* db, void* ws, const float* mean, const float* invstd, float* bn_partial, int* bn_nblk, int dtype,
diff --git a/bio_image_unet_amd/engine.py b/bio_image_unet_amd/engine.py
--- a/bio_image_unet_amd/engine.py
+++ b/bio_image_unet_amd/engine.py
@@ -29,6 +29,7 @@
 _NO_CAPTURE_FORK = _disabled("capturefork")
 _NO_SIDE_CHAIN = _disabled("sidechain")
 _NO_PREPACK = _disabled("prepack")
+_NO_HEAD_RANK1 = _disabled("headrank1") or _disabled("head_bnred")
 _SIDE_WGRAD_VOX = int(os.environ.get("BIU_SIDE_WGRAD_VOX", str(4 * 32 ** 3)))
 
 class Buf:
@@ -247,6 +248,7 @@
             yout.buf.producer[yout.leaves[0]] = self
         self.red_partial: Optional[torch.Tensor] = None
         self.red_nblk = 0
+        self.rank1 = None
         self.kd, self.kh, self.kw = _ksize(conv.weight)
         self.dil = int(conv.dilation[0])
         drop = seq[3] if len(seq) > 3 else None
@@ -448,7 +450,18 @@
         skip.mark_g()
         return deferred
 
+    def rank1_ok(self, eng, head_cout: int) -> bool:
+        if eng.trace or _NO_HEAD_RANK1 or eng.tdtype != torch.bfloat16 or not self.batch_stats:
+            return False
+        if self.foldt is not None or isinstance(self.xin, CatAct) or self.fold_wg:
+            return False
+        if self.kd == 3 and self.y.nvox <= _SIDE_WGRAD_VOX and eng.chain_stream() is not None:
+            return False
+        return bool(lib.biu_conv_bwd_weight_bn_rank1_ok(self.xin.a(), self.y.g(), self.y.a(), head_cout, self.kd, self.kh, self.kw, self.dil,
+                                                        eng.dtype))
+
     def bwd(self, eng):
+        rank1, self.rank1 = self.rank1, None
         if not self.y.g_written():
             return
         st = _stream()
@@ -510,6 +523,10 @@
             lib.label = label
             eng.defer_grads(done, [(self.conv.weight, dw)])
             dw = None
+        elif rank1 is not None:
+            check(lib.biu_conv_bwd_weight_bn_rank1(self.xin.a(), self.xin.xf(), _ptr(rank1[0]), _ptr(rank1[1]), 1, y.g(), y.a(), scale, shift,
+                                                   slope, _ptr(A), _ptr(B), _ptr(Cc), self.kd, self.kh, self.kw, self.dil, _ptr(dw),
+                                                   _ptr(eng.ws), eng.ws_bytes, eng.dtype, st), "conv_bwd_weight_bn_rank1")
         else:
             check(lib.biu_conv_bwd_weight_bn(self.xin.a(), self.xin.xf(), y.g(), y.a(), scale, shift, slope, _ptr(A), _ptr(B),
                                              _ptr(Cc), self.kd, self.kh, self.kw, self.dil, _ptr(dw), _ptr(eng.ws), eng.ws_bytes,
@@ -852,7 +869,7 @@
                                    _ptr(dst), ctot, c0, _stream()), "head_dlogits")
         return dst
 
-    def bwd_with(self, eng, dl: Optional[torch.Tensor]):
+    def bwd_with(self, eng, dl: Optional[torch.Tensor], logits_only: bool = False):
         if dl is None:
             return
         dl = dl.contiguous().float()
@@ -864,8 +881,11 @@
         if up is not None:
             part = up.red_buffer(eng, up.kd, 0)
             n_up = C.c_int(0)
+            rank1 = logits_only and self.cout == 1 and up.rank1_ok(eng, self.cout)
+            if rank1:
+                up.rank1 = (dl, self.conv.weight.data)
             check(lib.biu_head_bwd_bnred(self.xin.a(), self.xin.xf(), _ptr(self.conv.weight.data), self.cout, _ptr(dl),
-                                         self.xin.g(), _ptr(dw), _ptr(db), _ptr(eng.ws), eng.ws_bytes, _ptr(up.save_mean),
+                                         None if rank1 else self.xin.g(), _ptr(dw), _ptr(db), _ptr(eng.ws), eng.ws_bytes, _ptr(up.save_mean),
                                          _ptr(up.save_invstd), _ptr(part), part.numel(), C.byref(n_up), eng.dtype, st),
                   "head_bwd_bnred")
             up.red_nblk = n_up.value
@@ -1186,7 +1206,7 @@
     def _backward_head_group(self, live):
         if len(live) == 1:
             h, (gl, ga, a) = live[0]
-            h.bwd_with(self, h.dlogits(self, gl, ga, a))
+            h.bwd_with(self, h.dlogits(self, gl, ga, a), logits_only=ga is None)
             return
         x = live[0][0].xin
         assert all(h.xin is x for h, _ in live)
@@ -1271,6 +1291,7 @@
             outs.append(h.logits if kind == "logits" else h.activated)
         ctx.act_slot = {hi: i for i, (hi, kind) in enumerate(out_spec) if kind == "act"}
         ctx.save_for_backward(*[outs[i] for i in ctx.act_slot.values()])
+        ctx.set_materialize_grads(False)
         for h in eng.heads:
             h.logits = h.activated = None
         return tuple(outs)
diff --git a/include/biu.h b/include/biu.h
--- a/include/biu.h
+++ b/include/biu.h
@@ -88,6 +88,12 @@
                            const float* scale, const float* shift, const float* slope, const float* coefA,
                            const float* coefB, const float* coefC, int kd, int kh, int kw, int dilation,
                            float* dw, void* ws, size_t ws_bytes, int dtype, biu_stream stream);
+int biu_conv_bwd_weight_bn_rank1_ok(const biu_act* x, const biu_act* dy, const biu_act* y, int head_cout, int kd, int kh, int kw,
+                                    int dilation, int dtype);
+int biu_conv_bwd_weight_bn_rank1(const biu_act* x, const biu_xform* xf, const float* dlogits, const float* w_head, int head_cout,
+                                 const biu_act* dy, const biu_act* y, const float* scale, const float* shift, const float* slope,
+                                 const float* coefA, const float* coefB, const float* coefC, int kd, int kh, int kw, int dilation,
+                                 float* dw, void* ws, size_t ws_bytes, int dtype, biu_stream stream);
 
 #define BIU_BN_MAX_PARTIALS 1024
 int biu_bn_stats(const biu_act* y, float* partial, int* nblk_out, int dtype, biu_stream stream);
```

New measurement: 742.8 million voxels/s (median of 6 runs). 1.0% higher.
